# radoslawkrolikowski/financial-market-data-analysis

Measured on AMD Instinct MI355X. Metric: train seq/sec + 3-class acc, biGRU on synthetic order-book, higher is better.
Workload: dtype bf16; 1 GPU; model=biGRU L2 H128 bidirectional, global_batch=8192, seq_len=120, n_features=96, parallelism=dp1, bench_config=repo

## Files before the change

fmda_amd/ops/blas.py:

```python
import os


import torch

_TUNABLE_READY = False


def enable_tunableop() -> bool:
    global _TUNABLE_READY
    if _TUNABLE_READY or not torch.cuda.is_available():
        return _TUNABLE_READY
    try:
        tun = torch.cuda.tunable
        csv = os.path.join(os.path.dirname(__file__), "tunableop_gfx950.csv")
        tune = os.environ.get("FMDA_TUNE", "0") == "1"
        tun.set_filename(csv, insert_device_ordinal=False)
        tun.enable(True)
        tun.tuning_enable(tune)
        _TUNABLE_READY = True
    except Exception:
        _TUNABLE_READY = False
    return _TUNABLE_READY


def chunked_colsum(dg: torch.Tensor, chunks: int = 48) -> torch.Tensor:
    M, N = dg.shape
    c = chunks
    while c > 1 and M % c != 0:
        c //= 2
    if c <= 1:
        return dg.sum(dim=0, dtype=torch.float32)
    return dg.view(c, M // c, N).sum(dim=1, dtype=torch.float32).sum(dim=0)


def chunked_outer(dg: torch.Tensor, x: torch.Tensor,
                  chunks: int = 64, out_fp32: bool = False) -> torch.Tensor:
    M, N = dg.shape
    K = x.shape[1]
    c = chunks
    while c > 1 and M % c != 0:
        c //= 2
    if c <= 1:
        r = torch.matmul(dg.t(), x)
        return r.float() if out_fp32 else r
    parts = torch.bmm(dg.view(c, M // c, N).transpose(1, 2),
                      x.view(c, M // c, K))
    s = parts.float().sum(dim=0)
    return s if out_fp32 else s.to(dg.dtype)
```

fmda_amd/ops/csrc/bindings.cpp:

```cpp
#include <torch/extension.h>
#include <ATen/hip/HIPContext.h>

#include <vector>

extern "C" int fmda_gru_fwd_launch(int is_bf16, int Hp, const void* gi,
                                   const void* w, const float* bhh, void* out,
                                   float* hlast, int B, int Tseq, int n_dir,
                                   const float* h0, void* out_drop,
                                   unsigned int drop_thr, float drop_scale,
                                   unsigned long long drop_seed,
                                   hipStream_t stream);
extern "C" int fmda_gru_fwd_cs_launch(const void* gi, const void* w,
                                      const float* bhh, void* out,
                                      float* hlast, void* hpub,
                                      unsigned int* cnt, int B, int Tseq,
                                      int n_dir, void* out_drop,
                                      unsigned int drop_thr,
                                      float drop_scale,
                                      unsigned long long drop_seed,
                                      hipStream_t stream);
extern "C" int fmda_gru_bwd_cs_launch(const void* gi, const void* w,
                                      const void* wt, const float* bhh,
                                      const void* out, const void* dout,
                                      const float* dhT, void* dgi, void* dgh,
                                      float* dh0, float* dbhh, void* gpub,
                                      unsigned int* cnt, int B, int Tseq,
                                      int n_dir, unsigned int drop_thr,
                                      float drop_scale,
                                      unsigned long long drop_seed,
                                      hipStream_t stream);
extern "C" int fmda_gru_bwd_launch(int is_bf16, int Hp, const void* gi,
                                   const void* w, const void* wt,
                                   const float* bhh,
                                   const void* out, const void* dout,
                                   const float* dhT, void* dgi, void* dgh,
                                   float* dh0, float* dbhh, int B, int Tseq,
                                   int n_dir, unsigned int drop_thr,
                                   float drop_scale,
                                   unsigned long long drop_seed,
                                   const float* h0, void* dgh0,
                                   hipStream_t stream);
extern "C" int fmda_mfma_selftest_launch(const void* A, const void* Bm,
                                         float* C, hipStream_t stream);
extern "C" int fmda_pool_fwd_launch(int is_bf16, const void* out, float* maxv,
                                    float* avgv, int* amax, int B, int Tseq,
                                    int H, int n_dir, hipStream_t stream);
extern "C" int fmda_pool_bwd_launch(int is_bf16, const float* dmax,
                                    const float* davg, const int* amax,
                                    void* dout, int B, int Tseq, int H,
                                    int n_dir, hipStream_t stream);
extern "C" int fmda_dropout_launch(int is_bf16, const void* x, void* y,
                                   long n, unsigned int thr, float scale,
                                   unsigned long long seed,
                                   hipStream_t stream);
extern "C" int fmda_spatial_dropout_launch(int is_bf16, const void* x,
                                           void* y, long B, long Tlen, long F,
                                           unsigned int thr, float scale,
                                           unsigned long long seed,
                                           hipStream_t stream);
extern "C" int fmda_ingest_row_launch(void* ring, const float* row,
                                      const float* xmin, const float* xrng,
                                      int Tseq, int F, hipStream_t stream);
extern "C" int fmda_pool_concat_launch(int is_bf16, const void* out,
                                       const float* hlast, void* feat, int B,
                                       int Tseq, int H, int Hp, int n_dir,
                                       hipStream_t stream);
extern "C" int fmda_head_sigmoid_launch(int is_bf16, const void* x,
                                        const void* W, const void* bias,
                                        float* probs, int B, int K, int C,
                                        hipStream_t stream);
extern "C" int fmda_head_fwd_launch(int is_bf16, const void* x, const void* W,
                                    const void* bias, const float* y,
                                    const float* wgt, const float* pw,
                                    float* logits, float* sig,
                                    float* loss_sum, int B, int K, int C,
                                    hipStream_t stream);
extern "C" int fmda_head_bwd_launch(int is_bf16, const float* sig,
                                    const float* y, const float* wgt,
                                    const float* pw, const float* gscale,
                                    const void* W, float* dlogits, void* dx,
                                    int B, int K, int C, hipStream_t stream);
extern "C" int fmda_gru_bwd_db_rows(int is_bf16, int Hp, int B,
                                    int column_split);
extern "C" int fmda_gru_db_reduce_launch(const float* part, int rows,
                                         int n_dir, int Hp, float* dbhh,
                                         float* dbih, hipStream_t stream);
extern "C" int fmda_opt_norm2_launch(const void* chunks, int n_chunks,
                                     float* out, hipStream_t stream);
namespace fmda_ckpt {
void save_state_dict(const std::string& path,
                     const std::vector<std::string>& keys,
                     const std::vector<torch::Tensor>& tensors);
std::vector<std::pair<std::string, torch::Tensor>> load_state_dict(
        const std::string& path);
}

extern "C" int fmda_opt_adam_launch(const void* chunks, int n_chunks,
                                    const float* norm2, float clip, float lr,
                                    float beta1, float beta2, float eps,
                                    float bc1, float bc2, hipStream_t stream);

namespace {

void check_common(const torch::Tensor& gi, const torch::Tensor& w,
                  const torch::Tensor& bhh, int& B, int& T, int& n_dir,
                  int& Hp, bool& is_bf16) {
    TORCH_CHECK(gi.is_cuda() && w.is_cuda() && bhh.is_cuda(),
                "fmda gru: tensors must be on GPU");
    TORCH_CHECK(gi.is_contiguous() && w.is_contiguous() && bhh.is_contiguous(),
                "fmda gru: tensors must be contiguous");
    TORCH_CHECK(gi.dim() == 3 && w.dim() == 3, "fmda gru: bad ranks");
    TORCH_CHECK(w.scalar_type() == gi.scalar_type(), "fmda gru: dtype mismatch");
    TORCH_CHECK(bhh.scalar_type() == torch::kFloat32, "bhh must be fp32");
    n_dir = w.size(0);
    Hp = w.size(2);
    TORCH_CHECK(w.size(1) == 3 * Hp, "w must be (n_dir, 3H, H)");
    B = gi.size(0);
    T = gi.size(1);
    TORCH_CHECK(gi.size(2) == (int64_t)n_dir * 3 * Hp, "gi last dim mismatch");
    TORCH_CHECK(n_dir == 1 || n_dir == 2, "n_dir must be 1 or 2");
    is_bf16 = gi.scalar_type() == torch::kBFloat16;
    TORCH_CHECK(is_bf16 || gi.scalar_type() == torch::kFloat32,
                "fmda gru: dtype must be bf16 or fp32");
    TORCH_CHECK(!(is_bf16 && Hp < 32),
                "fmda gru: bf16 requires Hp >= 32 (MFMA K=32); pad the "
                "hidden size");
}

struct DropParams {
    unsigned int thr;
    float scale;
};

DropParams drop_params(double p) {
    if (!(p > 0.0)) return {0u, 1.0f};
    return {(unsigned int)((float)p * 256.0f), (float)(1.0 / (1.0 - p))};
}

}

std::vector<torch::Tensor> gru_fwd(torch::Tensor gi, torch::Tensor w,
                                   torch::Tensor bhh,
                                   c10::optional<torch::Tensor> h0_opt,
                                   double drop_p, int64_t drop_seed) {
    int B, T, n_dir, Hp;
    bool is_bf16;
    check_common(gi, w, bhh, B, T, n_dir, Hp, is_bf16);
    const float* h0 = nullptr;
    if (h0_opt.has_value()) {
        auto& h = h0_opt.value();
        TORCH_CHECK(h.is_cuda() && h.is_contiguous() &&
                    h.scalar_type() == torch::kFloat32 &&
                    h.sizes() == torch::IntArrayRef({n_dir, B, Hp}),
                    "h0 must be contiguous fp32 (n_dir, B, Hp)");
        h0 = h.data_ptr<float>();
    }
    auto out = torch::empty({B, T, (int64_t)n_dir * Hp}, gi.options());
    auto hlast = torch::empty({n_dir, B, Hp},
                              gi.options().dtype(torch::kFloat32));
    const DropParams dp = drop_params(drop_p);
    const unsigned int drop_thr = dp.thr;
    const float drop_scale = dp.scale;
    torch::Tensor out_drop;
    void* out_drop_ptr = nullptr;
    if (drop_thr != 0u) {
        TORCH_CHECK(is_bf16 && (Hp == 128 || Hp == 512),
                    "fused fwd dropout requires bf16 Hp=128/512");
        TORCH_CHECK(Hp == 128 || h0 == nullptr,
                    "fused fwd dropout with h0 requires Hp=128");
        out_drop = torch::empty_like(out);
        out_drop_ptr = out_drop.data_ptr();
    }
    auto stream = at::hip::getCurrentHIPStream();
    int rc;
    if (is_bf16 && Hp == 512 && h0 == nullptr) {
        const int BR = 256;
        const int GB = (B + BR - 1) / BR;
        const int G = GB * n_dir;
        auto hpub = torch::empty({2, G, BR, (int64_t)Hp}, gi.options());
        auto cnt = torch::zeros({G}, gi.options().dtype(torch::kUInt32));
        rc = fmda_gru_fwd_cs_launch(gi.data_ptr(), w.data_ptr(),
                                    bhh.data_ptr<float>(), out.data_ptr(),
                                    hlast.data_ptr<float>(), hpub.data_ptr(),
                                    (unsigned int*)cnt.data_ptr(), B, T,
                                    n_dir, out_drop_ptr, drop_thr,
                                    drop_scale,
                                    (unsigned long long)drop_seed,
                                    stream.stream());
    } else {
        rc = fmda_gru_fwd_launch(is_bf16 ? 1 : 0, Hp, gi.data_ptr(),
                                 w.data_ptr(), bhh.data_ptr<float>(),
                                 out.data_ptr(), hlast.data_ptr<float>(), B, T,
                                 n_dir, h0, out_drop_ptr, drop_thr,
                                 drop_scale,
                                 (unsigned long long)drop_seed,
                                 stream.stream());
    }
    TORCH_CHECK(rc == 0, "fmda gru_fwd launch failed rc=", rc, " Hp=", Hp);
    if (out_drop_ptr != nullptr)
        return {out, hlast, out_drop};
    return {out, hlast};
}

std::vector<torch::Tensor> gru_bwd(torch::Tensor gi, torch::Tensor w,
                                   torch::Tensor bhh, torch::Tensor out,
                                   torch::Tensor dout, torch::Tensor dhT,
                                   double drop_p, int64_t drop_seed,
                                   c10::optional<torch::Tensor> h0_opt) {
    int B, T, n_dir, Hp;
    bool is_bf16;
    check_common(gi, w, bhh, B, T, n_dir, Hp, is_bf16);
    const float* h0 = nullptr;
    torch::Tensor dgh0;
    void* dgh0_ptr = nullptr;
    if (h0_opt.has_value()) {
        auto& h = h0_opt.value();
        TORCH_CHECK(h.is_cuda() && h.is_contiguous() &&
                    h.scalar_type() == torch::kFloat32 &&
                    h.sizes() == torch::IntArrayRef({n_dir, B, Hp}),
                    "h0 must be contiguous fp32 (n_dir, B, Hp)");
        h0 = h.data_ptr<float>();
        dgh0 = torch::empty({n_dir, B, (int64_t)3 * Hp}, gi.options());
        dgh0_ptr = dgh0.data_ptr();
    }
    TORCH_CHECK(out.is_contiguous() && dout.is_contiguous() &&
                dhT.is_contiguous(), "fmda gru_bwd: tensors must be contiguous");
    TORCH_CHECK(dhT.scalar_type() == torch::kFloat32, "dhT must be fp32");
    TORCH_CHECK(is_bf16 || Hp <= 256,
                "fp32 backward unsupported for Hp > 256 (LDS budget); "
                "train in bf16 for hidden sizes above 256");
    torch::Tensor dgi, dgh;
    if (getenv("FMDA_ZERO_GRADS")) {
        dgi = torch::zeros_like(gi);
        dgh = torch::zeros_like(gi);
    } else {
        dgi = torch::empty_like(gi);
        dgh = torch::empty_like(gi);
    }
    auto dh0 = torch::empty({n_dir, B, Hp},
                            gi.options().dtype(torch::kFloat32));
    const bool column_split = is_bf16 && Hp == 512 && h0 == nullptr;
    const int64_t db_rows = fmda_gru_bwd_db_rows(is_bf16 ? 1 : 0, Hp, B,
                                                 column_split ? 1 : 0);
    auto dbpart = torch::zeros({db_rows, n_dir, 4 * Hp},
                               gi.options().dtype(torch::kFloat32));
    torch::Tensor wt;
    const void* wt_ptr = nullptr;
    if (is_bf16 && (Hp == 128 || Hp == 512)) {
        wt = w.transpose(1, 2).contiguous();
        wt_ptr = wt.data_ptr();
    }
    auto stream = at::hip::getCurrentHIPStream();
    int rc;
    const DropParams dp = drop_params(drop_p);
    if (column_split) {
        const unsigned int cs_thr = dp.thr;
        const float cs_scale = dp.scale;
        const int BR = 256;
        const int GB = (B + BR - 1) / BR;
        const int G = GB * n_dir;
        auto gpub = torch::empty({2, G, BR, (int64_t)3 * Hp}, gi.options());
        auto cnt = torch::zeros({G}, gi.options().dtype(torch::kUInt32));
        rc = fmda_gru_bwd_cs_launch(
            gi.data_ptr(), w.data_ptr(), wt_ptr, bhh.data_ptr<float>(),
            out.data_ptr(), dout.data_ptr(), dhT.data_ptr<float>(),
            dgi.data_ptr(), dgh.data_ptr(), dh0.data_ptr<float>(),
            dbpart.data_ptr<float>(), gpub.data_ptr(),
            (unsigned int*)cnt.data_ptr(), B, T, n_dir, cs_thr, cs_scale,
            (unsigned long long)drop_seed, stream.stream());
    } else {
        const unsigned int drop_thr = dp.thr;
        const float drop_scale = dp.scale;
        TORCH_CHECK(drop_thr == 0u || (is_bf16 && Hp == 128),
                    "fused dropout-backward on this path requires bf16 "
                    "Hp=128");
        rc = fmda_gru_bwd_launch(is_bf16 ? 1 : 0, Hp, gi.data_ptr(),
                                 w.data_ptr(), wt_ptr, bhh.data_ptr<float>(),
                                 out.data_ptr(), dout.data_ptr(),
                                 dhT.data_ptr<float>(), dgi.data_ptr(),
                                 dgh.data_ptr(), dh0.data_ptr<float>(),
                                 dbpart.data_ptr<float>(), B, T,
                                 n_dir, drop_thr, drop_scale,
                                 (unsigned long long)drop_seed, h0, dgh0_ptr,
                                 stream.stream());
    }
    TORCH_CHECK(rc == 0, "fmda gru_bwd launch failed rc=", rc, " Hp=", Hp);
    auto dbhh = torch::empty({n_dir, 3 * Hp},
                             gi.options().dtype(torch::kFloat32));
    auto dbih = torch::empty_like(dbhh);
    rc = fmda_gru_db_reduce_launch(dbpart.data_ptr<float>(), (int)db_rows,
                                   n_dir, Hp, dbhh.data_ptr<float>(),
                                   dbih.data_ptr<float>(), stream.stream());
    TORCH_CHECK(rc == 0, "fmda gru db reduce launch failed");
    if (dgh0_ptr != nullptr)
        return {dgi, dgh, dh0, dbhh, dbih, dgh0};
    return {dgi, dgh, dh0, dbhh, dbih};
}

torch::Tensor mfma_selftest(torch::Tensor A, torch::Tensor Bm) {
    TORCH_CHECK(A.is_cuda() && A.scalar_type() == torch::kBFloat16);
    TORCH_CHECK(A.sizes() == torch::IntArrayRef({16, 32}) &&
                Bm.sizes() == torch::IntArrayRef({32, 16}));
    auto C = torch::empty({16, 16}, A.options().dtype(torch::kFloat32));
    auto stream = at::hip::getCurrentHIPStream();
    int rc = fmda_mfma_selftest_launch(A.contiguous().data_ptr(),
                                       Bm.contiguous().data_ptr(),
                                       C.data_ptr<float>(), stream.stream());
    TORCH_CHECK(rc == 0, "mfma selftest launch failed");
    return C;
}

std::vector<torch::Tensor> pool_fwd(torch::Tensor out, int64_t n_dir) {
    TORCH_CHECK(out.is_cuda() && out.is_contiguous() && out.dim() == 3);
    const bool bf16 = out.scalar_type() == torch::kBFloat16;
    TORCH_CHECK(bf16 || out.scalar_type() == torch::kFloat32);
    const int B = out.size(0), T = out.size(1);
    const int H = out.size(2) / n_dir;
    TORCH_CHECK(H % 2 == 0, "pool_fwd pairs columns: H must be even "
                "(odd H uses the eager path)");
    auto f32 = out.options().dtype(torch::kFloat32);
    auto maxv = torch::empty({B, H}, f32);
    auto avgv = torch::empty({B, H}, f32);
    auto amax = torch::empty({B, H}, out.options().dtype(torch::kInt32));
    auto stream = at::hip::getCurrentHIPStream();
    int rc = fmda_pool_fwd_launch(bf16 ? 1 : 0, out.data_ptr(),
                                  maxv.data_ptr<float>(), avgv.data_ptr<float>(),
                                  amax.data_ptr<int>(), B, T, H, (int)n_dir,
                                  stream.stream());
    TORCH_CHECK(rc == 0, "pool_fwd launch failed");
    return {maxv, avgv, amax};
}

torch::Tensor pool_bwd(torch::Tensor dmax, torch::Tensor davg,
                       torch::Tensor amax, int64_t T, int64_t n_dir,
                       torch::ScalarType dtype) {
    TORCH_CHECK(dmax.is_cuda() && dmax.is_contiguous() && davg.is_contiguous());
    const int B = dmax.size(0), H = dmax.size(1);
    const bool bf16 = dtype == torch::kBFloat16;
    auto dout = torch::empty({B, T, n_dir * H}, dmax.options().dtype(dtype));
    auto stream = at::hip::getCurrentHIPStream();
    int rc = fmda_pool_bwd_launch(bf16 ? 1 : 0, dmax.data_ptr<float>(),
                                  davg.data_ptr<float>(), amax.data_ptr<int>(),
                                  dout.data_ptr(), B, (int)T, H, (int)n_dir,
                                  stream.stream());
    TORCH_CHECK(rc == 0, "pool_bwd launch failed");
    return dout;
}

torch::Tensor fused_clip_adam(torch::Tensor chunks, int64_t n_chunks,
                              double clip, double lr, double beta1,
                              double beta2, double eps, int64_t step) {
    TORCH_CHECK(chunks.is_cuda() && chunks.scalar_type() == torch::kInt64);
    auto f32 = chunks.options().dtype(torch::kFloat32);
    torch::Tensor norm2;
    auto stream = at::hip::getCurrentHIPStream();
    if (clip > 0) {
        auto part = torch::empty({std::min<int64_t>(n_chunks, 2048)}, f32);
        int rc = fmda_opt_norm2_launch(chunks.data_ptr(), (int)n_chunks,
                                       part.data_ptr<float>(),
                                       stream.stream());
        TORCH_CHECK(rc == 0, "opt norm2 launch failed");
        norm2 = part.sum().reshape({1});
    } else {
        norm2 = torch::zeros({1}, f32);
    }
    const float bc1 = 1.0f - powf((float)beta1, (float)step);
    const float bc2 = 1.0f - powf((float)beta2, (float)step);
    int rc = fmda_opt_adam_launch(chunks.data_ptr(), (int)n_chunks,
                                  norm2.data_ptr<float>(), (float)clip,
                                  (float)lr, (float)beta1, (float)beta2,
                                  (float)eps, bc1, bc2, stream.stream());
    TORCH_CHECK(rc == 0, "opt adam launch failed");
    return norm2;
}

std::vector<torch::Tensor> head_loss_fwd(torch::Tensor x, torch::Tensor W,
                                         torch::Tensor b, torch::Tensor y,
                                         torch::Tensor wgt, torch::Tensor pw) {
    TORCH_CHECK(x.is_cuda() && x.is_contiguous() && W.is_contiguous());
    const bool bf16 = x.scalar_type() == torch::kBFloat16;
    const int B = x.size(0), K = x.size(1), C = W.size(0);
    auto f32 = x.options().dtype(torch::kFloat32);
    auto logits = torch::empty({B, C}, f32);
    auto sig = torch::empty({B, C}, f32);
    auto part = torch::empty({((int64_t)B * C + 255) / 256}, f32);
    auto stream = at::hip::getCurrentHIPStream();
    int rc = fmda_head_fwd_launch(
        bf16 ? 1 : 0, x.data_ptr(), W.data_ptr(), b.data_ptr(),
        y.data_ptr<float>(), wgt.data_ptr<float>(), pw.data_ptr<float>(),
        logits.data_ptr<float>(), sig.data_ptr<float>(),
        part.data_ptr<float>(), B, K, C, stream.stream());
    TORCH_CHECK(rc == 0, "head fwd launch failed");
    return {logits, sig, part.sum().reshape({1})};
}

std::vector<torch::Tensor> head_loss_bwd(torch::Tensor sig, torch::Tensor y,
                                         torch::Tensor wgt, torch::Tensor pw,
                                         torch::Tensor gscale,
                                         torch::Tensor W,
                                         torch::ScalarType xdtype) {
    const int B = sig.size(0), C = sig.size(1), K = W.size(1);
    const bool bf16 = xdtype == torch::kBFloat16;
    auto dlogits = torch::empty_like(sig);
    auto dx = torch::empty({B, K}, sig.options().dtype(xdtype));
    auto stream = at::hip::getCurrentHIPStream();
    int rc = fmda_head_bwd_launch(
        bf16 ? 1 : 0, sig.data_ptr<float>(), y.data_ptr<float>(),
        wgt.data_ptr<float>(), pw.data_ptr<float>(),
        gscale.data_ptr<float>(), W.data_ptr(), dlogits.data_ptr<float>(),
        dx.data_ptr(), B, K, C, stream.stream());
    TORCH_CHECK(rc == 0, "head bwd launch failed");
    return {dlogits, dx};
}

torch::Tensor dropout_fused(torch::Tensor x, double p, int64_t seed) {
    TORCH_CHECK(x.is_cuda() && x.is_contiguous() &&
                x.scalar_type() == torch::kBFloat16);
    auto y = torch::empty_like(x);
    auto stream = at::hip::getCurrentHIPStream();
    const DropParams dp = drop_params(p);
    int rc = fmda_dropout_launch(1, x.data_ptr(), y.data_ptr(), x.numel(),
                                 dp.thr, dp.scale, (unsigned long long)seed,
                                 stream.stream());
    TORCH_CHECK(rc == 0, "dropout launch failed");
    return y;
}

torch::Tensor spatial_dropout_fused(torch::Tensor x, double p,
                                    int64_t seed) {
    TORCH_CHECK(x.is_cuda() && x.is_contiguous() && x.dim() == 3 &&
                x.scalar_type() == torch::kBFloat16);
    auto y = torch::empty_like(x);
    auto stream = at::hip::getCurrentHIPStream();
    const DropParams dp = drop_params(p);
    int rc = fmda_spatial_dropout_launch(
        1, x.data_ptr(), y.data_ptr(), x.size(0), x.size(1), x.size(2),
        dp.thr, dp.scale, (unsigned long long)seed, stream.stream());
    TORCH_CHECK(rc == 0, "spatial dropout launch failed");
    return y;
}

void ingest_row(torch::Tensor ring, torch::Tensor row, torch::Tensor xmin,
                torch::Tensor xrng) {
    TORCH_CHECK(ring.is_cuda() && ring.is_contiguous() && ring.dim() == 2 &&
                ring.scalar_type() == torch::kBFloat16,
                "ring must be (T, F) bf16 on GPU");
    TORCH_CHECK(row.is_cuda() && row.is_contiguous() &&
                row.scalar_type() == torch::kFloat32 &&
                row.numel() == ring.size(1));
    TORCH_CHECK(xmin.is_cuda() && xmin.is_contiguous() &&
                xmin.scalar_type() == torch::kFloat32 &&
                xmin.numel() == ring.size(1), "xmin must be fp32 (F) on GPU");
    TORCH_CHECK(xrng.is_cuda() && xrng.is_contiguous() &&
                xrng.scalar_type() == torch::kFloat32 &&
                xrng.numel() == ring.size(1), "xrng must be fp32 (F) on GPU");
    auto stream = at::hip::getCurrentHIPStream();
    int rc = fmda_ingest_row_launch(
        ring.data_ptr(), row.data_ptr<float>(), xmin.data_ptr<float>(),
        xrng.data_ptr<float>(), ring.size(0), ring.size(1), stream.stream());
    TORCH_CHECK(rc == 0, "ingest_row launch failed rc=", rc);
}

torch::Tensor pool_concat_infer(torch::Tensor out, torch::Tensor hlast,
                                int64_t H) {
    TORCH_CHECK(out.is_cuda() && out.is_contiguous() && out.dim() == 3);
    TORCH_CHECK(hlast.is_contiguous() &&
                hlast.scalar_type() == torch::kFloat32);
    const bool bf16 = out.scalar_type() == torch::kBFloat16;
    const int B = out.size(0), T = out.size(1);
    const int n_dir = hlast.size(0);
    const int Hp = hlast.size(2);
    auto feat = torch::empty({B, 3 * H}, out.options());
    auto stream = at::hip::getCurrentHIPStream();
    int rc = fmda_pool_concat_launch(bf16 ? 1 : 0, out.data_ptr(),
                                     hlast.data_ptr<float>(), feat.data_ptr(),
                                     B, T, (int)H, Hp, n_dir,
                                     stream.stream());
    TORCH_CHECK(rc == 0, "pool_concat launch failed");
    return feat;
}

torch::Tensor head_sigmoid(torch::Tensor x, torch::Tensor W,
                           torch::Tensor b) {
    TORCH_CHECK(x.is_cuda() && x.is_contiguous() && W.is_contiguous() &&
                b.is_contiguous());
    TORCH_CHECK(x.scalar_type() == W.scalar_type() &&
                x.scalar_type() == b.scalar_type());
    const bool bf16 = x.scalar_type() == torch::kBFloat16;
    const int B = x.size(0), K = x.size(1), C = W.size(0);
    auto probs = torch::empty({B, C}, x.options().dtype(torch::kFloat32));
    auto stream = at::hip::getCurrentHIPStream();
    int rc = fmda_head_sigmoid_launch(bf16 ? 1 : 0, x.data_ptr(),
                                      W.data_ptr(), b.data_ptr(),
                                      probs.data_ptr<float>(), B, K, C,
                                      stream.stream());
    TORCH_CHECK(rc == 0, "head_sigmoid launch failed");
    return probs;
}

PYBIND11_MODULE(TORCH_EXTENSION_NAME, m) {
    m.def("gru_fwd", &gru_fwd, "fused biGRU recurrence forward (HIP/CDNA4)",
          py::arg("gi"), py::arg("w"), py::arg("bhh"),
          py::arg("h0") = py::none(), py::arg("drop_p") = 0.0,
          py::arg("drop_seed") = 0);
    m.def("gru_bwd", &gru_bwd, "fused biGRU recurrence backward (HIP/CDNA4)",
          py::arg("gi"), py::arg("w"), py::arg("bhh"), py::arg("out"),
          py::arg("dout"), py::arg("dhT"), py::arg("drop_p") = 0.0,
          py::arg("drop_seed") = 0, py::arg("h0") = py::none());
    m.def("mfma_selftest", &mfma_selftest, "mfma fragment layout self-test");
    m.def("dropout_fused", &dropout_fused,
          "counter-based dropout (mask recomputed in backward)");
    m.def("spatial_dropout_fused", &spatial_dropout_fused,
          "channel (Dropout2d) dropout over (B, T, F) without permutes");
    m.def("ingest_row", &ingest_row,
          "streaming ingest: shift GPU window ring + normalize new row");
    m.def("pool_concat_infer", &pool_concat_infer,
          "fused [dirsum(h_last) | max | avg] concat for inference");
    m.def("head_sigmoid", &head_sigmoid,
          "linear head + sigmoid emitting probabilities");
    m.def("pool_fwd", &pool_fwd, "fused dirsum+max/avg pooling forward");
    m.def("pool_bwd", &pool_bwd, "fused pooling backward (d_out assembly)");
    m.def("head_loss_fwd", &head_loss_fwd, "fused head GEMM + BCE loss");
    m.def("head_loss_bwd", &head_loss_bwd, "fused head/loss backward");
    m.def("fused_clip_adam", &fused_clip_adam,
          "fused multi-tensor grad-clip + Adam step");
    m.def("save_state_dict_native", &fmda_ckpt::save_state_dict,
          "write a torch.load-compatible zip state_dict (native C++)");
    m.def("load_state_dict_native", &fmda_ckpt::load_state_dict,
          "read a torch.save zip state_dict (native C++)");
}
```

fmda_amd/ops/csrc/gru_kernels.hip:

```cpp
#include <hip/hip_runtime.h>
#include <hip/hip_bf16.h>

#define FMDA_DEV __device__ __forceinline__

typedef __bf16 bf16x8_t __attribute__((ext_vector_type(8)));
typedef float f32x4_t __attribute__((ext_vector_type(4)));

namespace fmda {

#define FMDA_LOG2E 1.4426950408889634f

FMDA_DEV float fast_exp2(float x) { return __builtin_amdgcn_exp2f(x); }
FMDA_DEV float fast_rcp(float x) { return __builtin_amdgcn_rcpf(x); }

FMDA_DEV float sigmoidf(float x) {
    return fast_rcp(1.0f + fast_exp2(-x * FMDA_LOG2E));
}

FMDA_DEV float fast_tanh(float x) {
    return 1.0f - 2.0f * fast_rcp(1.0f + fast_exp2(2.0f * FMDA_LOG2E * x));
}

template <typename T> FMDA_DEV float to_f32(T v);
template <> FMDA_DEV float to_f32<float>(float v) { return v; }
// ... 1925 lines not shown
                        (const bf16x8_t*)(asrc + (long)row * 3 * Hp + kbase));
                }
#pragma unroll
                for (int j = 0; j < JT; ++j) {
                    const bf16x8_t bfr = *(const bf16x8_t*)&(
                        (const __bf16*)wt_dir)[
                        (long)(ct * CS + j * 16 + (lane & 15)) * 3 * Hp +
                        kbase];
#pragma unroll
                    for (int m = 0; m < MT; ++m)
                        acc2[j][m] = __builtin_amdgcn_mfma_f32_16x16x32_bf16(
                            a[m], bfr, acc2[j][m], 0, 0, 0);
                }
            }
#pragma unroll
            for (int j = 0; j < JT; ++j)
#pragma unroll
                for (int m = 0; m < MT; ++m)
#pragma unroll
                    for (int e = 0; e < 4; ++e)
                        dhcar[j][m][e] += acc2[j][m][e];
        }

        const bool haveh = (u > 0);
        const __hip_bfloat16* hsrc =
            out_b + (long)(rev ? (Tseq - u) : (u - 1)) * n_dir * Hp;
        f32x4_t acc[NCT][MT];
#pragma unroll
        for (int i = 0; i < NCT; ++i)
#pragma unroll
            for (int m = 0; m < MT; ++m) acc[i][m] = f32x4_t{0.f};
        if (haveh) {
            const int arow = lane & 15;
            const int koff = 8 * (lane >> 4);
#pragma unroll
            for (int kk = 0; kk < KK; ++kk) {
                const int kbase = 32 * kk + koff;
                bf16x8_t a[MT];
#pragma unroll
                for (int m = 0; m < MT; ++m) {
                    int row = 16 * (wave + NW * m) + arow;
                    if (row >= rows_valid) row = 0;
                    a[m] = *(const bf16x8_t*)(hsrc + (long)row * out_row +
                                              kbase);
                }
#pragma unroll
                for (int i = 0; i < NCT; ++i) {
                    const bf16x8_t b = *(const bf16x8_t*)&(
                        (const __bf16*)w_s)[(i * 16 + (lane & 15)) * WPITCH +
                                            kbase];
#pragma unroll
                    for (int m = 0; m < MT; ++m)
                        acc[i][m] = __builtin_amdgcn_mfma_f32_16x16x32_bf16(
                            a[m], b, acc[i][m], 0, 0, 0);
                }
            }
        }

        const __hip_bfloat16* do_t = dout_b + (long)tt * n_dir * Hp + ct * CS;
        float keep_dhn[JT][MT][4];
#pragma unroll
        for (int j = 0; j < JT; ++j) {
            const int jj = j * 16 + (lane & 15);
#pragma unroll
            for (int m = 0; m < MT; ++m) {
#pragma unroll
                for (int e = 0; e < 4; ++e) {
                    const int b = 16 * (wave + NW * m) + 4 * (lane >> 4) + e;
                    const bool live = (b < rows_valid);
                    const float gr = acc[j][m][e] + bhh_s[jj];
                    const float gz = acc[JT + j][m][e] + bhh_s[CS + jj];
                    const float hn =
                        acc[2 * JT + j][m][e] + bhh_s[2 * CS + jj];
                    const float ir = (float)((const __bf16*)gi_s)[b * GP + jj];
                    const float iz =
                        (float)((const __bf16*)gi_s)[b * GP + CS + jj];
                    const float in_ =
                        (float)((const __bf16*)gi_s)[b * GP + 2 * CS + jj];
                    const float r = sigmoidf(ir + gr);
                    const float z = sigmoidf(iz + gz);
                    const float n = fast_tanh(in_ + r * hn);
                    const float hprev =
                        (live && haveh)
                            ? (float)hsrc[(long)b * out_row + ct * CS + jj]
                            : 0.0f;
                    float doval =
                        live ? (float)do_t[(long)b * out_row + jj] : 0.0f;
                    if (drop_thr != 0u) {
                        const long o = ((long)(b0 + b) * Tseq + tt) *
                                           n_dir * Hp +
                                       (long)dir * Hp + ct * CS + jj;
                        const unsigned long long rnd =
                            mix64(drop_seed ^ (unsigned long long)(o >> 3));
                        const unsigned int u =
                            (unsigned int)(rnd >> (8 * ((int)o & 7))) & 0xFF;
                        doval = (u < drop_thr) ? 0.0f : doval * drop_scale;
                    }
                    const float dht = dhcar[j][m][e] + doval;
                    const float dz_pre =
                        live ? dht * (hprev - n) * z * (1.0f - z) : 0.0f;
                    const float dn_pre =
                        live ? dht * (1.0f - z) * (1.0f - n * n) : 0.0f;
                    const float dr_pre =
                        live ? dn_pre * hn * r * (1.0f - r) : 0.0f;
                    const float dhn = live ? dn_pre * r : 0.0f;
                    ((__bf16*)gi_s)[b * GP + jj] =
                        (__bf16)__float2bfloat16(dr_pre);
                    ((__bf16*)gi_s)[b * GP + CS + jj] =
                        (__bf16)__float2bfloat16(dz_pre);
                    ((__bf16*)gi_s)[b * GP + 2 * CS + jj] =
                        (__bf16)__float2bfloat16(dn_pre);
                    keep_dhn[j][m][e] = dhn;
                    dhcar[j][m][e] = live ? dht * z : 0.0f;
                    dbacc[j][0] += dr_pre;
                    dbacc[j][1] += dz_pre;
                    dbacc[j][2] += dhn;
                    dbacc[j][3] += dn_pre;
                }
            }
        }
        asm volatile("s_waitcnt lgkmcnt(0)" ::: "memory");
        __syncthreads();

        {
            __hip_bfloat16* dst = dgi_b + (long)tt * n_dir * 3 * Hp;
            for (int g3 = 0; g3 < 3; ++g3)
                store_tile<__hip_bfloat16, BR, NT>(
                    gi_s + g3 * CS, dst + g3 * Hp + ct * CS, CS, GP, gi_row,
                    rows_valid, tid);
        }
        asm volatile("s_waitcnt lgkmcnt(0)" ::: "memory");
        __syncthreads();
#pragma unroll
        for (int j = 0; j < JT; ++j) {
            const int jj = j * 16 + (lane & 15);
#pragma unroll
            for (int m = 0; m < MT; ++m)
#pragma unroll
                for (int e = 0; e < 4; ++e) {
                    const int b = 16 * (wave + NW * m) + 4 * (lane >> 4) + e;
                    ((__bf16*)gi_s)[b * GP + 2 * CS + jj] =
                        (__bf16)__float2bfloat16(keep_dhn[j][m][e]);
                }
        }
        asm volatile("s_waitcnt lgkmcnt(0)" ::: "memory");
        __syncthreads();
        {
            const int sh = rev ? (tt + 1) : (tt - 1);
            if (sh >= 0 && sh < Tseq) {
                __hip_bfloat16* dst = dgh_b + (long)sh * n_dir * 3 * Hp;
                for (int g3 = 0; g3 < 3; ++g3)
                    store_tile<__hip_bfloat16, BR, NT>(
                        gi_s + g3 * CS, dst + g3 * Hp + ct * CS, CS, GP,
                        gi_row, rows_valid, tid);
            } else {
                __hip_bfloat16* dst =
                    dgh_b + (long)(rev ? 0 : (Tseq - 1)) * n_dir * 3 * Hp;
                for (int g3 = 0; g3 < 3; ++g3)
                    store_zero_tile<__hip_bfloat16, BR, NT>(
                        dst + g3 * Hp + ct * CS, CS, gi_row, rows_valid, tid);
            }
            if (u > 0) {
                __hip_bfloat16* dst =
                    pub_base + (long)(u & 1) * ring_stride;
                constexpr int CPR = CS * 2 / 16;
                for (int g3 = 0; g3 < 3; ++g3)
                    for (int c = tid; c < BR * CPR; c += NT) {
                        const int r = c / CPR;
                        const int jc = c % CPR;
                        u32x4_t v = *(const u32x4_t*)((const char*)(gi_s +
                                        g3 * CS) + (long)r * GP * 2 + jc * 16);
                        store16_sc1((char*)(dst + (long)r * 3 * Hp +
                                            g3 * Hp + ct * CS) + jc * 16, v);
                    }
                asm volatile("s_waitcnt vmcnt(0)" ::: "memory");
                __syncthreads();
                if (tid == 0)
                    __hip_atomic_fetch_add(&cnt[g], 1u, __ATOMIC_RELAXED,
                                           __HIP_MEMORY_SCOPE_AGENT);
            }
        }
        if (u > 0)
            stage_gi(rev ? (Tseq - u) : (u - 1));
        asm volatile("s_waitcnt lgkmcnt(0)" ::: "memory");
        __syncthreads();
    }

    {
        float* d0 = dh0 + ((long)dir * B + b0) * Hp + ct * CS;
#pragma unroll
        for (int j = 0; j < JT; ++j) {
            const int jj = j * 16 + (lane & 15);
#pragma unroll
            for (int m = 0; m < MT; ++m)
#pragma unroll
                for (int e = 0; e < 4; ++e) {
                    const int b = 16 * (wave + NW * m) + 4 * (lane >> 4) + e;
                    if (b < rows_valid) d0[(long)b * Hp + jj] = dhcar[j][m][e];
                }
        }
        float* dbrow =
            dbhh + (((long)gb * NW + wave) * n_dir + dir) * 4 * Hp;
#pragma unroll
        for (int j = 0; j < JT; ++j)
#pragma unroll
            for (int q4 = 0; q4 < 4; ++q4) {
                float v = dbacc[j][q4];
                v += __shfl_xor(v, 16);
                v += __shfl_xor(v, 32);
                if ((lane >> 4) == 0)
                    dbrow[q4 * Hp + ct * CS + j * 16 + (lane & 15)] = v;
            }
    }
}


template <typename T>
__global__ void dropout_kernel(const T* __restrict__ x, T* __restrict__ y,
                               long n, unsigned int thr, float scale,
                               unsigned long long seed) {
    const long o = ((long)blockIdx.x * blockDim.x + threadIdx.x) * 8;
    if (o >= n) return;
    const unsigned long long r = mix64(seed ^ (unsigned long long)(o >> 3));
    if (o + 8 <= n) {
        T v[8];
        *(chunk16*)v = *(const chunk16*)(x + o);
#pragma unroll
        for (int k = 0; k < 8; ++k) {
            const unsigned int u = (unsigned int)(r >> (8 * k)) & 0xFF;
            v[k] = (u < thr) ? from_f32<T>(0.0f)
                             : from_f32<T>(to_f32<T>(v[k]) * scale);
        }
        *(chunk16*)(y + o) = *(const chunk16*)v;
    } else {
        for (long i = o; i < n; ++i) {
            const unsigned int u =
                (unsigned int)(r >> (8 * (i - o))) & 0xFF;
            y[i] = (u < thr) ? from_f32<T>(0.0f)
                             : from_f32<T>(to_f32<T>(x[i]) * scale);
        }
    }
}

extern "C" int fmda_dropout_launch(int is_bf16, const void* x, void* y,
                                   long n, unsigned int thr, float scale,
                                   unsigned long long seed,
                                   hipStream_t stream) {
    const long threads = (n + 7) / 8;
    const dim3 grid((threads + 255) / 256);
    if (is_bf16)
        dropout_kernel<__hip_bfloat16><<<grid, 256, 0, stream>>>(
            (const __hip_bfloat16*)x, (__hip_bfloat16*)y, n, thr, scale,
            seed);
    else
        return -2;
    return hipGetLastError() == hipSuccess ? 0 : -1;
}

template <typename T>
__global__ void spatial_dropout_kernel(const T* __restrict__ x,
                                       T* __restrict__ y, long n, long TF,
                                       int F, unsigned int thr, float scale,
                                       unsigned long long seed) {
    const long o = ((long)blockIdx.x * blockDim.x + threadIdx.x) * 8;
    if (o >= n) return;
    const int cnt = (int)((o + 8 <= n) ? 8 : (n - o));
    T v[8];
    if (cnt == 8)
        *(chunk16*)v = *(const chunk16*)(x + o);
    else
        for (int k = 0; k < cnt; ++k) v[k] = x[o + k];
#pragma unroll
    for (int k = 0; k < 8; ++k) {
        if (k >= cnt) break;
        const long i = o + k;
        const long c = (i / TF) * F + (i % F);
        const unsigned long long r =
            mix64(seed ^ (unsigned long long)(c >> 3));
        const unsigned int u = (unsigned int)(r >> (8 * ((int)c & 7))) & 0xFF;
        v[k] = (u < thr) ? from_f32<T>(0.0f)
                         : from_f32<T>(to_f32<T>(v[k]) * scale);
    }
    if (cnt == 8)
        *(chunk16*)(y + o) = *(const chunk16*)v;
    else
        for (int k = 0; k < cnt; ++k) y[o + k] = v[k];
}

extern "C" int fmda_spatial_dropout_launch(int is_bf16, const void* x,
                                           void* y, long B, long Tlen, long F,
                                           unsigned int thr, float scale,
                                           unsigned long long seed,
                                           hipStream_t stream) {
    if (!is_bf16) return -2;
    const long n = B * Tlen * F;
    const long threads = (n + 7) / 8;
    const dim3 grid((threads + 255) / 256);
    spatial_dropout_kernel<__hip_bfloat16><<<grid, 256, 0, stream>>>(
        (const __hip_bfloat16*)x, (__hip_bfloat16*)y, n, Tlen * F, (int)F,
        thr, scale, seed);
    return hipGetLastError() == hipSuccess ? 0 : -1;
}

template <typename T>
__global__ void pool_fwd_kernel(const T* __restrict__ out,
                                float* __restrict__ maxv,
                                float* __restrict__ avgv,
                                int* __restrict__ amax, int B, int Tseq,
                                int H, int n_dir) {
    const int idx = blockIdx.x * blockDim.x + threadIdx.x;
    const int HP2 = H / 2;
    if (idx >= B * HP2) return;
    const int b = idx / HP2;
    const int h2 = (idx % HP2) * 2;
    const int HD = n_dir * H;
    const T* p = out + (long)b * Tseq * HD + h2;
    float mx0 = -3.4e38f, mx1 = -3.4e38f, s0 = 0.0f, s1 = 0.0f;
    int im0 = 0, im1 = 0;
    for (int t = 0; t < Tseq; ++t) {
        const T* pt = p + (long)t * HD;
        struct alignas(2 * sizeof(T)) Pair { T x, y; };
        const Pair v2 = *(const Pair*)pt;
        float v0 = to_f32<T>(v2.x), v1 = to_f32<T>(v2.y);
        if (n_dir == 2) {
            const Pair w2 = *(const Pair*)(pt + H);
            v0 += to_f32<T>(w2.x);
            v1 += to_f32<T>(w2.y);
        }
        s0 += v0; s1 += v1;
        if (v0 > mx0) { mx0 = v0; im0 = t; }
        if (v1 > mx1) { mx1 = v1; im1 = t; }
    }
    const int o = b * H + h2;
    maxv[o] = mx0; maxv[o + 1] = mx1;
    avgv[o] = s0 / (float)Tseq; avgv[o + 1] = s1 / (float)Tseq;
    amax[o] = im0; amax[o + 1] = im1;
}

template <typename T>
__global__ void pool_bwd_kernel(const float* __restrict__ dmax,
                                const float* __restrict__ davg,
                                const int* __restrict__ amax,
                                T* __restrict__ dout, int B, int Tseq, int H,
                                int n_dir) {
    const int idx = blockIdx.x * blockDim.x + threadIdx.x;
    if (idx >= B * H) return;
    const int b = idx / H;
    const int h = idx % H;
    const int HD = n_dir * H;
    const float ga = davg[idx] / (float)Tseq;
    const float gm = dmax[idx];
    const int im = amax[idx];
    T* p = dout + (long)b * Tseq * HD + h;
    for (int t = 0; t < Tseq; ++t) {
        const float g = ga + (t == im ? gm : 0.0f);
        p[(long)t * HD] = from_f32<T>(g);
        if (n_dir == 2) p[(long)t * HD + H] = from_f32<T>(g);
    }
}

__global__ void pool_fwd_oct_kernel(const __hip_bfloat16* __restrict__ out,
                                    float* __restrict__ maxv,
                                    float* __restrict__ avgv,
                                    int* __restrict__ amax, int B, int Tseq,
                                    int H, int n_dir) {
    const int idx = blockIdx.x * blockDim.x + threadIdx.x;
    const int H8 = H / 8;
    if (idx >= B * H8) return;
    const int b = idx / H8;
    const int h8 = (idx % H8) * 8;
    const int HD = n_dir * H;
    const __hip_bfloat16* p = out + (long)b * Tseq * HD + h8;
    float mx[8], s[8];
    int im[8];
#pragma unroll
    for (int k = 0; k < 8; ++k) { mx[k] = -3.4e38f; s[k] = 0.0f; im[k] = 0; }
    for (int t = 0; t < Tseq; ++t) {
        const __hip_bfloat16* pt = p + (long)t * HD;
        bf16x8_t v = *(const bf16x8_t*)pt;
        bf16x8_t w;
        if (n_dir == 2) w = *(const bf16x8_t*)(pt + H);
#pragma unroll
        for (int k = 0; k < 8; ++k) {
            float x = (float)((const __bf16*)&v)[k];
            if (n_dir == 2) x += (float)((const __bf16*)&w)[k];
            s[k] += x;
            if (x > mx[k]) { mx[k] = x; im[k] = t; }
        }
    }
    const int o = b * H + h8;
#pragma unroll
    for (int k = 0; k < 8; ++k) {
        maxv[o + k] = mx[k];
        avgv[o + k] = s[k] / (float)Tseq;
        amax[o + k] = im[k];
    }
}

__global__ void pool_bwd_oct_kernel(const float* __restrict__ dmax,
                                    const float* __restrict__ davg,
                                    const int* __restrict__ amax,
                                    __hip_bfloat16* __restrict__ dout,
                                    int B, int Tseq, int H, int n_dir) {
    const int idx = blockIdx.x * blockDim.x + threadIdx.x;
    const int H8 = H / 8;
    if (idx >= B * H8) return;
    const int b = idx / H8;
    const int h8 = (idx % H8) * 8;
    const int o = b * H + h8;
    float ga[8], gm[8];
    int im[8];
#pragma unroll
    for (int k = 0; k < 8; ++k) {
        ga[k] = davg[o + k] / (float)Tseq;
        gm[k] = dmax[o + k];
        im[k] = amax[o + k];
    }
    const int HD = n_dir * H;
    __hip_bfloat16* p = dout + (long)b * Tseq * HD + h8;
    for (int t = 0; t < Tseq; ++t) {
        bf16x8_t v;
#pragma unroll
        for (int k = 0; k < 8; ++k)
            ((__bf16*)&v)[k] =
                (__bf16)__float2bfloat16(ga[k] + (t == im[k] ? gm[k] : 0.0f));
        *(bf16x8_t*)(p + (long)t * HD) = v;
        if (n_dir == 2) *(bf16x8_t*)(p + (long)t * HD + H) = v;
    }
}

template <typename T>
__global__ void pool_fwd_small_kernel(const T* __restrict__ out,
                                      float* __restrict__ maxv,
                                      float* __restrict__ avgv,
                                      int* __restrict__ amax, int B, int Tseq,
                                      int H, int n_dir) {
    const int HP2 = H / 2;
    const int wave = threadIdx.x >> 6;
    const int lane = threadIdx.x & 63;
    const int idx = blockIdx.x * (blockDim.x >> 6) + wave;
    if (idx >= B * HP2) return;
    const int b = idx / HP2;
    const int h2 = (idx % HP2) * 2;
    const int HD = n_dir * H;
    const T* p = out + (long)b * Tseq * HD + h2;
    float mx0 = -3.4e38f, mx1 = -3.4e38f, s0 = 0.0f, s1 = 0.0f;
    int im0 = Tseq, im1 = Tseq;
    for (int t = lane; t < Tseq; t += 64) {
        const T* pt = p + (long)t * HD;
        struct alignas(2 * sizeof(T)) Pair { T x, y; };
        const Pair v2 = *(const Pair*)pt;
        float v0 = to_f32<T>(v2.x), v1 = to_f32<T>(v2.y);
        if (n_dir == 2) {
            const Pair w2 = *(const Pair*)(pt + H);
            v0 += to_f32<T>(w2.x);
            v1 += to_f32<T>(w2.y);
        }
        s0 += v0; s1 += v1;
        if (v0 > mx0) { mx0 = v0; im0 = t; }
        if (v1 > mx1) { mx1 = v1; im1 = t; }
    }
#pragma unroll
    for (int d = 1; d < 64; d <<= 1) {
        const float omx0 = __shfl_xor(mx0, d), omx1 = __shfl_xor(mx1, d);
        const int oim0 = __shfl_xor(im0, d), oim1 = __shfl_xor(im1, d);
        s0 += __shfl_xor(s0, d);
        s1 += __shfl_xor(s1, d);
        if (omx0 > mx0 || (omx0 == mx0 && oim0 < im0)) { mx0 = omx0; im0 = oim0; }
        if (omx1 > mx1 || (omx1 == mx1 && oim1 < im1)) { mx1 = omx1; im1 = oim1; }
    }
    if (lane == 0) {
        const int o = b * H + h2;
        maxv[o] = mx0; maxv[o + 1] = mx1;
        avgv[o] = s0 / (float)Tseq; avgv[o + 1] = s1 / (float)Tseq;
        amax[o] = im0; amax[o + 1] = im1;
    }
}

extern "C" int fmda_pool_fwd_launch(int is_bf16, const void* out, float* maxv,
                                    float* avgv, int* amax, int B, int Tseq,
                                    int H, int n_dir, hipStream_t stream) {
    const int n = B * (H / 2);
    if (n < 4096) {
        const dim3 grid((n + 3) / 4);
        if (is_bf16)
            pool_fwd_small_kernel<__hip_bfloat16><<<grid, 256, 0, stream>>>(
                (const __hip_bfloat16*)out, maxv, avgv, amax, B, Tseq, H,
                n_dir);
        else
            pool_fwd_small_kernel<float><<<grid, 256, 0, stream>>>(
                (const float*)out, maxv, avgv, amax, B, Tseq, H, n_dir);
        return hipGetLastError() == hipSuccess ? 0 : -1;
    }
    if (is_bf16 && H % 8 == 0) {
        const int n8 = B * (H / 8);
        pool_fwd_oct_kernel<<<dim3((n8 + 255) / 256), 256, 0, stream>>>(
            (const __hip_bfloat16*)out, maxv, avgv, amax, B, Tseq, H, n_dir);
        return hipGetLastError() == hipSuccess ? 0 : -1;
    }
    const dim3 grid((n + 255) / 256);
    if (is_bf16)
        pool_fwd_kernel<__hip_bfloat16><<<grid, 256, 0, stream>>>(
            (const __hip_bfloat16*)out, maxv, avgv, amax, B, Tseq, H, n_dir);
    else
        pool_fwd_kernel<float><<<grid, 256, 0, stream>>>(
            (const float*)out, maxv, avgv, amax, B, Tseq, H, n_dir);
    return hipGetLastError() == hipSuccess ? 0 : -1;
}

extern "C" int fmda_pool_bwd_launch(int is_bf16, const float* dmax,
                                    const float* davg, const int* amax,
                                    void* dout, int B, int Tseq, int H,
                                    int n_dir, hipStream_t stream) {
    const int n = B * H;
    if (is_bf16 && H % 8 == 0 && B * (H / 8) >= 4096) {
        const int n8 = B * (H / 8);
        pool_bwd_oct_kernel<<<dim3((n8 + 255) / 256), 256, 0, stream>>>(
            dmax, davg, amax, (__hip_bfloat16*)dout, B, Tseq, H, n_dir);
        return hipGetLastError() == hipSuccess ? 0 : -1;
    }
    const dim3 grid((n + 255) / 256);
    if (is_bf16)
        pool_bwd_kernel<__hip_bfloat16><<<grid, 256, 0, stream>>>(
            dmax, davg, amax, (__hip_bfloat16*)dout, B, Tseq, H, n_dir);
    else
        pool_bwd_kernel<float><<<grid, 256, 0, stream>>>(
            dmax, davg, amax, (float*)dout, B, Tseq, H, n_dir);
    return hipGetLastError() == hipSuccess ? 0 : -1;
}


__global__ void ingest_row_kernel(__hip_bfloat16* __restrict__ ring,
                                  const float* __restrict__ row,
                                  const float* __restrict__ xmin,
                                  const float* __restrict__ xrng,
                                  int Tseq, int F) {
    const int n = (Tseq - 1) * F;
    const int tid = threadIdx.x;
    __hip_bfloat16 keep[48];
    int cnt = 0;
    for (int i = tid; i < n; i += blockDim.x) keep[cnt++] = ring[i + F];
    __syncthreads();
    cnt = 0;
    for (int i = tid; i < n; i += blockDim.x) ring[i] = keep[cnt++];
    for (int f = tid; f < F; f += blockDim.x)
        ring[n + f] = __float2bfloat16((row[f] - xmin[f]) / xrng[f]);
}

extern "C" int fmda_ingest_row_launch(void* ring, const float* row,
                                      const float* xmin, const float* xrng,
                                      int Tseq, int F, hipStream_t stream) {
    const int n = (Tseq - 1) * F;
    if (n > 48 * 1024) return -5;
    ingest_row_kernel<<<1, 1024, 0, stream>>>(
        (__hip_bfloat16*)ring, row, xmin, xrng, Tseq, F);
    return hipGetLastError() == hipSuccess ? 0 : -1;
}

template <typename T>
__global__ void pool_concat_infer_kernel(const T* __restrict__ out,
                                         const float* __restrict__ hlast,
                                         T* __restrict__ feat, int B,
                                         int Tseq, int H, int Hp, int n_dir) {
    const int HP2 = H / 2;
    const int wave = threadIdx.x >> 6;
    const int lane = threadIdx.x & 63;
    const int idx = blockIdx.x * (blockDim.x >> 6) + wave;
    if (idx >= B * HP2) return;
    const int b = idx / HP2;
    const int h2 = (idx % HP2) * 2;
    const int HD = n_dir * H;
    const T* p = out + (long)b * Tseq * HD + h2;
    float mx0 = -3.4e38f, mx1 = -3.4e38f, s0 = 0.0f, s1 = 0.0f;
    for (int t = lane; t < Tseq; t += 64) {
        const T* pt = p + (long)t * HD;
        struct alignas(2 * sizeof(T)) Pair { T x, y; };
        const Pair v2 = *(const Pair*)pt;
        float v0 = to_f32<T>(v2.x), v1 = to_f32<T>(v2.y);
        if (n_dir == 2) {
            const Pair w2 = *(const Pair*)(pt + H);
            v0 += to_f32<T>(w2.x);
            v1 += to_f32<T>(w2.y);
        }
        s0 += v0; s1 += v1;
        if (v0 > mx0) mx0 = v0;
        if (v1 > mx1) mx1 = v1;
    }
#pragma unroll
    for (int d = 1; d < 64; d <<= 1) {
        const float omx0 = __shfl_xor(mx0, d), omx1 = __shfl_xor(mx1, d);
        s0 += __shfl_xor(s0, d);
        s1 += __shfl_xor(s1, d);
        if (omx0 > mx0) mx0 = omx0;
        if (omx1 > mx1) mx1 = omx1;
    }
    if (lane == 0) {
        float hl0 = hlast[(long)b * Hp + h2];
        float hl1 = hlast[(long)b * Hp + h2 + 1];
        if (n_dir == 2) {
            hl0 += hlast[((long)B + b) * Hp + h2];
            hl1 += hlast[((long)B + b) * Hp + h2 + 1];
        }
        T* fr = feat + (long)b * 3 * H;
        fr[h2] = from_f32<T>(hl0);
        fr[h2 + 1] = from_f32<T>(hl1);
        fr[H + h2] = from_f32<T>(mx0);
        fr[H + h2 + 1] = from_f32<T>(mx1);
        fr[2 * H + h2] = from_f32<T>(s0 / (float)Tseq);
        fr[2 * H + h2 + 1] = from_f32<T>(s1 / (float)Tseq);
    }
}

extern "C" int fmda_pool_concat_launch(int is_bf16, const void* out,
                                       const float* hlast, void* feat, int B,
                                       int Tseq, int H, int Hp, int n_dir,
                                       hipStream_t stream) {
    const int n = B * (H / 2);
    const dim3 grid((n + 3) / 4);
    if (is_bf16)
        pool_concat_infer_kernel<__hip_bfloat16><<<grid, 256, 0, stream>>>(
            (const __hip_bfloat16*)out, hlast, (__hip_bfloat16*)feat, B,
            Tseq, H, Hp, n_dir);
    else
        pool_concat_infer_kernel<float><<<grid, 256, 0, stream>>>(
            (const float*)out, hlast, (float*)feat, B, Tseq, H, Hp, n_dir);
    return hipGetLastError() == hipSuccess ? 0 : -1;
}

template <typename T>
__global__ void head_sigmoid_kernel(const T* __restrict__ x,
                                    const T* __restrict__ W,
                                    const T* __restrict__ bias,
                                    float* __restrict__ probs, int B, int K,
                                    int C) {
    const int wave = threadIdx.x >> 6;
    const int lane = threadIdx.x & 63;
    const int idx = blockIdx.x * (blockDim.x >> 6) + wave;
    if (idx >= B * C) return;
    const int b = idx / C, c = idx % C;
    const T* xr = x + (long)b * K;
    const T* wr = W + (long)c * K;
    float acc = 0.0f;
    for (int k = lane; k < K; k += 64)
        acc += to_f32<T>(xr[k]) * to_f32<T>(wr[k]);
#pragma unroll
    for (int d = 1; d < 64; d <<= 1) acc += __shfl_xor(acc, d);
    if (lane == 0) probs[idx] = sigmoidf(acc + to_f32<T>(bias[c]));
}

extern "C" int fmda_head_sigmoid_launch(int is_bf16, const void* x,
                                        const void* W, const void* bias,
                                        float* probs, int B, int K, int C,
                                        hipStream_t stream) {
    const int n = B * C;
    const dim3 grid((n + 3) / 4);
    if (is_bf16)
        head_sigmoid_kernel<__hip_bfloat16><<<grid, 256, 0, stream>>>(
            (const __hip_bfloat16*)x, (const __hip_bfloat16*)W,
            (const __hip_bfloat16*)bias, probs, B, K, C);
    else
        head_sigmoid_kernel<float><<<grid, 256, 0, stream>>>(
            (const float*)x, (const float*)W, (const float*)bias, probs, B,
            K, C);
    return hipGetLastError() == hipSuccess ? 0 : -1;
}

template <typename T>
__global__ void head_loss_fwd_kernel(const T* __restrict__ x,
                                     const T* __restrict__ W,
                                     const T* __restrict__ bias,
                                     const float* __restrict__ y,
                                     const float* __restrict__ wgt,
                                     const float* __restrict__ pw,
                                     float* __restrict__ logits,
                                     float* __restrict__ sig,
                                     float* __restrict__ loss_sum, int B,
                                     int K, int C) {
    const int idx = blockIdx.x * blockDim.x + threadIdx.x;
    float l = 0.0f;
    if (idx < B * C) {
        const int r = idx / C, c = idx % C;
        const T* xr = x + (long)r * K;
        const T* wr = W + (long)c * K;
        float acc = to_f32<T>(bias[c]);
        for (int k = 0; k < K; ++k)
            acc += to_f32<T>(xr[k]) * to_f32<T>(wr[k]);
        logits[idx] = acc;
        const float s = sigmoidf(acc);
        sig[idx] = s;
        const float yy = y[idx];
        const float m = acc > 0.0f ? acc : 0.0f;
        const float lse = m + __builtin_logf(fast_exp2(-m * FMDA_LOG2E) +
                                             fast_exp2((acc - m) * FMDA_LOG2E));
        const float log_s = acc - lse;
        const float log_1ms = -lse;
        l = -wgt[c] * (pw[c] * yy * log_s + (1.0f - yy) * log_1ms);
    }
    __shared__ float red[4];
    float v = l;
    v += __shfl_xor(v, 1); v += __shfl_xor(v, 2); v += __shfl_xor(v, 4);
    v += __shfl_xor(v, 8); v += __shfl_xor(v, 16); v += __shfl_xor(v, 32);
    if ((threadIdx.x & 63) == 0) red[threadIdx.x >> 6] = v;
    __syncthreads();
    if (threadIdx.x == 0) {
        float t = 0.0f;
        for (int w = 0; w < (int)(blockDim.x >> 6); ++w) t += red[w];
        loss_sum[blockIdx.x] = t;
    }
}

template <typename T>
__global__ void head_loss_bwd_kernel(const float* __restrict__ sig,
                                     const float* __restrict__ y,
                                     const float* __restrict__ wgt,
                                     const float* __restrict__ pw,
                                     const float* __restrict__ gscale,
                                     const T* __restrict__ W,
                                     float* __restrict__ dlogits,
                                     T* __restrict__ dx, int B, int K, int C) {
    const int idx = blockIdx.x * blockDim.x + threadIdx.x;
    if (idx >= B * K) return;
    const int r = idx / K, k = idx % K;
    const float g = *gscale / (float)(B * C);
    float acc = 0.0f;
    for (int c = 0; c < C; ++c) {
        const float s = sig[r * C + c];
        const float yy = y[r * C + c];
        const float dl = g * wgt[c] * (s * (1.0f - yy + pw[c] * yy) -
                                       pw[c] * yy);
        if (k == 0) dlogits[r * C + c] = dl;
        acc += dl * to_f32<T>(W[(long)c * K + k]);
    }
    dx[idx] = from_f32<T>(acc);
}

extern "C" int fmda_head_fwd_launch(int is_bf16, const void* x, const void* W,
                                    const void* bias, const float* y,
                                    const float* wgt, const float* pw,
                                    float* logits, float* sig,
                                    float* loss_sum, int B, int K, int C,
                                    hipStream_t stream) {
    const int n = B * C;
    const dim3 grid((n + 255) / 256);
    if (is_bf16)
        head_loss_fwd_kernel<__hip_bfloat16><<<grid, 256, 0, stream>>>(
            (const __hip_bfloat16*)x, (const __hip_bfloat16*)W,
            (const __hip_bfloat16*)bias, y, wgt, pw, logits, sig, loss_sum,
            B, K, C);
    else
        head_loss_fwd_kernel<float><<<grid, 256, 0, stream>>>(
            (const float*)x, (const float*)W, (const float*)bias, y, wgt, pw,
            logits, sig, loss_sum, B, K, C);
    return hipGetLastError() == hipSuccess ? 0 : -1;
}

extern "C" int fmda_head_bwd_launch(int is_bf16, const float* sig,
                                    const float* y, const float* wgt,
                                    const float* pw, const float* gscale,
                                    const void* W, float* dlogits, void* dx,
                                    int B, int K, int C, hipStream_t stream) {
    const int n = B * K;
    const dim3 grid((n + 255) / 256);
    if (is_bf16)
        head_loss_bwd_kernel<__hip_bfloat16><<<grid, 256, 0, stream>>>(
            sig, y, wgt, pw, gscale, (const __hip_bfloat16*)W, dlogits,
            (__hip_bfloat16*)dx, B, K, C);
    else
        head_loss_bwd_kernel<float><<<grid, 256, 0, stream>>>(
            sig, y, wgt, pw, gscale, (const float*)W, dlogits, (float*)dx,
            B, K, C);
    return hipGetLastError() == hipSuccess ? 0 : -1;
}

__global__ void mfma_selftest_kernel(const __hip_bfloat16* __restrict__ A,
                                     const __hip_bfloat16* __restrict__ Bm,
                                     float* __restrict__ C) {
    const int lane = threadIdx.x & 63;
    bf16x8_t a, b;
    const __bf16* ap = (const __bf16*)A;
    const __bf16* bp = (const __bf16*)Bm;
#pragma unroll
    for (int e = 0; e < 8; ++e) {
        a[e] = ap[(lane & 15) * 32 + 8 * (lane >> 4) + e];
        b[e] = bp[(8 * (lane >> 4) + e) * 16 + (lane & 15)];
    }
    f32x4_t acc = f32x4_t{0.f};
    acc = __builtin_amdgcn_mfma_f32_16x16x32_bf16(a, b, acc, 0, 0, 0);
#pragma unroll
    for (int v = 0; v < 4; ++v)
        C[(4 * (lane >> 4) + v) * 16 + (lane & 15)] = acc[v];
}


struct LaunchCfg { int bt; bool wlds; int nt; bool hoist; };

static inline LaunchCfg fwd_cfg(bool bf16, int Hp) {
    if (bf16) {
        if (Hp <= 64) return {32, true, 256, false};
        if (Hp == 128) return {32, false, 512, true};
        if (Hp == 256) return {32, false, 512, false};
        return {16, false, 512, false};
    }
    if (Hp <= 128) return {32, false, 256, false};
    return {16, false, 256, false};
}
static inline LaunchCfg bwd_cfg(bool bf16, int Hp) {
    if (bf16) {
        if (Hp <= 64) return {32, true, 256, false};
        if (Hp == 128) return {32, false, 512, true};
        if (Hp == 256) return {32, false, 512, false};
        return {16, false, 512, false};
    }
    if (Hp <= 128) return {32, false, 256, false};
    return {16, false, 256, false};
}

static inline size_t fwd_lds_bytes(bool bf16, int Hp, int bt, bool wlds) {
    const size_t es = bf16 ? 2 : 4;
    const size_t pade = 16 / es;
    const size_t wp = Hp + pade, gp3 = 3 * Hp + pade, hfp = Hp + 4;
    size_t s = 0;
    if (wlds) s += es * 3 * Hp * wp;
    s += 4 * (size_t)bt * hfp;
    if (bf16) s += 2 * (size_t)bt * wp;
    s += es * (size_t)bt * gp3;
    s += 4 * (size_t)3 * Hp;
    return s;
}
static inline size_t bwd_lds_bytes(bool bf16, int Hp, int bt, bool wlds) {
    const size_t es = bf16 ? 2 : 4;
// ... 376 lines not shown
```

fmda_amd/ops/interface.py:

```python
import os
from typing import List, Optional, Tuple

import torch

from . import load_extension
from .blas import chunked_colsum, chunked_outer, enable_tunableop

_ALLOWED_HP = [32, 64, 128, 256, 512]


def _pad_h(H: int) -> int:
    for hp in _ALLOWED_HP:
        if H <= hp:
            return hp
    raise ValueError(f"hidden size {H} > {_ALLOWED_HP[-1]} not supported")


def _pad_gate_rows(w: torch.Tensor, H: int, Hp: int) -> torch.Tensor:
    if H == Hp:
        return w
    shape = list(w.shape)
    shape[0] = 3 * Hp
    out = w.new_zeros(shape)
    for g in range(3):
        out[g * Hp:g * Hp + H] = w[g * H:(g + 1) * H]
    return out


def _pad_cols(w: torch.Tensor, H: int, Hp: int) -> torch.Tensor:
    if H == Hp:
        return w
    shape = list(w.shape)
    shape[-1] = Hp
    out = w.new_zeros(shape)
    out[..., :H] = w
    return out


class _GRURecurrence(torch.autograd.Function):

    @staticmethod
    def forward(ctx, gi, w, bhh, h0=None):
        ext = load_extension()
        gi = gi.contiguous()
        w = w.contiguous()
        bhh32 = bhh.to(torch.float32).contiguous()
        h0c = (h0.detach().to(torch.float32).contiguous()
               if h0 is not None else None)
        out, h_last = ext.gru_fwd(gi, w, bhh32, h0c)
        ctx.save_for_backward(gi, w, bhh32, out)
        ctx.h0 = h0c
        return out, h_last

    @staticmethod
    def backward(ctx, d_out, d_hlast):
        ext = load_extension()
        gi, w, bhh32, out = ctx.saved_tensors
        h0c = ctx.h0
        B, T, _ = gi.shape
        n_dir, threeHp, Hp = w.shape
        d_out = d_out.contiguous().to(gi.dtype)
        d_hlast = d_hlast.contiguous().to(torch.float32)
        res = ext.gru_bwd(gi, w, bhh32, out, d_out, d_hlast, 0.0, 0, h0c)
        dgi, dgh, dh0_out, dbhh, _dbih = res[:5]
        dgh0 = res[5] if len(res) > 5 else None

        cross = chunked_outer(dgh.reshape(-1, n_dir * threeHp),
                              out.reshape(-1, n_dir * Hp))
        dw = torch.empty_like(w)
        for d in range(n_dir):
            dw[d] = cross[d * threeHp:(d + 1) * threeHp,
                          d * Hp:(d + 1) * Hp]
            if dgh0 is not None:
                dw[d] += (dgh0[d].float().t() @ h0c[d]).to(dw.dtype)
        dh0_grad = dh0_out if h0c is not None else None
        return dgi, dw, dbhh, dh0_grad


def gru_directions(gi: torch.Tensor, w: torch.Tensor, bhh: torch.Tensor,
                   h0: Optional[torch.Tensor] = None
                   ) -> Tuple[torch.Tensor, torch.Tensor]:
    return _GRURecurrence.apply(gi, w, bhh, h0)


class _IHProjection(torch.autograd.Function):

    @staticmethod
    def forward(ctx, x2d, w, b):
        ctx.save_for_backward(x2d, w)
        return torch.addmm(b, x2d, w.t())

    @staticmethod
    def backward(ctx, dgi):
        x2d, w = ctx.saved_tensors
        dgi = dgi.contiguous()
        dx = dw = db = None
        if ctx.needs_input_grad[0]:
            dx = torch.matmul(dgi, w)
        if ctx.needs_input_grad[1]:
            dw = chunked_outer(dgi, x2d)
        if ctx.needs_input_grad[2]:
            db = chunked_colsum(dgi).to(dgi.dtype)
        return dx, dw, db


class _FusedDropout(torch.autograd.Function):

    @staticmethod
    def forward(ctx, x, p, seed):
        ext = load_extension()
        ctx.p = p
        ctx.seed = seed
        return ext.dropout_fused(x.contiguous(), p, seed)

    @staticmethod
    def backward(ctx, dy):
        ext = load_extension()
        return ext.dropout_fused(dy.contiguous(), ctx.p, ctx.seed), None, None


def fused_dropout(x: torch.Tensor, p: float) -> torch.Tensor:
    if not (x.is_cuda and x.dtype == torch.bfloat16 and 0.0 < p < 1.0):
        return torch.nn.functional.dropout(x, p=p, training=True)
    seed = int(torch.empty((), dtype=torch.int64).random_())
    return _FusedDropout.apply(x, p, seed)


class _FusedSpatialDropout(torch.autograd.Function):

    @staticmethod
    def forward(ctx, x, p, seed):
        ext = load_extension()
        ctx.p = p
        ctx.seed = seed
        return ext.spatial_dropout_fused(x.contiguous(), p, seed)

    @staticmethod
    def backward(ctx, dy):
        ext = load_extension()
        return (ext.spatial_dropout_fused(dy.contiguous(), ctx.p, ctx.seed),
                None, None)


def fused_spatial_dropout(x: torch.Tensor, p: float) -> torch.Tensor:
    if not (x.is_cuda and x.dtype == torch.bfloat16 and 0.0 < p < 1.0):
        y = torch.nn.functional.dropout2d(
            x.permute(0, 2, 1).unsqueeze(-1), p=p, training=True)
        return y.squeeze(-1).permute(0, 2, 1)
    seed = int(torch.empty((), dtype=torch.int64).random_())
    return _FusedSpatialDropout.apply(x, p, seed)


class _DirSumPool(torch.autograd.Function):

    @staticmethod
    def forward(ctx, out, n_dir):
        ext = load_extension()
        out = out.contiguous()
        maxv, avgv, amax = ext.pool_fwd(out, n_dir)
        ctx.save_for_backward(amax)
        ctx.meta = (out.shape[1], n_dir, out.dtype)
        return maxv.to(out.dtype), avgv.to(out.dtype)

    @staticmethod
    def backward(ctx, dmax, davg):
        ext = load_extension()
        (amax,) = ctx.saved_tensors
        T, n_dir, dtype = ctx.meta
        dout = ext.pool_bwd(dmax.float().contiguous(),
                            davg.float().contiguous(), amax, T, n_dir, dtype)
        return dout, None


def dirsum_pool(out: torch.Tensor, n_dir: int):
    return _DirSumPool.apply(out, n_dir)


class _HeadLoss(torch.autograd.Function):

    @staticmethod
    def forward(ctx, x2d, W, b, y, wgt, pw):
        ext = load_extension()
        x2d = x2d.contiguous()
        logits, sig, loss_sum = ext.head_loss_fwd(
            x2d, W.contiguous(), b.contiguous(), y.contiguous(),
            wgt.contiguous(), pw.contiguous())
        B, C = logits.shape
        loss = (loss_sum / float(B * C)).reshape(())
        ctx.save_for_backward(x2d, W, y, wgt, pw, sig)
        ctx.mark_non_differentiable(logits)
        return loss, logits

    @staticmethod
    def backward(ctx, dloss, _dlogits):
        ext = load_extension()
        x2d, W, y, wgt, pw, sig = ctx.saved_tensors
        dlogits, dx = ext.head_loss_bwd(sig, y, wgt, pw,
                                        dloss.reshape(1).float().contiguous(),
                                        W, x2d.dtype)
        dl = dlogits.to(x2d.dtype)
        dW = chunked_outer(dl, x2d)
        db = dlogits.sum(dim=0).to(W.dtype)
        return dx, dW, db, None, None, None


def fused_head_loss(x2d, weight, bias, y, wgt, pw):
    Wc = weight.to(x2d.dtype)
    bc = bias.to(x2d.dtype)
    return _HeadLoss.apply(x2d, Wc, bc, y.float(), wgt.float(), pw.float())


def _unpad_gate_rows(w, H, Hp):
    if H == Hp:
        return w
    return torch.cat([w[g * Hp:g * Hp + H] for g in range(3)], dim=0)


class _BiGRULayer(torch.autograd.Function):

    @staticmethod
    def forward(ctx, x, Hp, w_ih0, w_hh0, b_ih0, b_hh0,
                w_ih1, w_hh1, b_ih1, b_hh1, out_drop_p=0.0,
                out_drop_seed=0, h0=None):
        ext = load_extension()
        D = 2 if w_ih1 is not None else 1
        H = w_hh0.shape[1]
        dtype = x.dtype
        B, T, F = x.shape
        with torch.no_grad():
            w_ihs = [_pad_gate_rows(w_ih0, H, Hp)]
            w_hhs = [_pad_cols(_pad_gate_rows(w_hh0, H, Hp), H, Hp)]
            b_ihs = [_pad_gate_rows(b_ih0, H, Hp)]
            b_hhs = [_pad_gate_rows(b_hh0, H, Hp)]
            if D == 2:
                w_ihs.append(_pad_gate_rows(w_ih1, H, Hp))
                w_hhs.append(_pad_cols(_pad_gate_rows(w_hh1, H, Hp), H, Hp))
                b_ihs.append(_pad_gate_rows(b_ih1, H, Hp))
                b_hhs.append(_pad_gate_rows(b_hh1, H, Hp))
            w_ih_cat = torch.cat(w_ihs, dim=0).to(dtype)
            b_ih_cat = torch.cat(b_ihs, dim=0).to(dtype)
            w_hh_cat = torch.stack(w_hhs, dim=0).to(dtype)
            b_hh_cat = torch.stack(b_hhs, dim=0).float()
        x2d = x.reshape(B * T, F)
        gi = torch.addmm(b_ih_cat, x2d, w_ih_cat.t()).view(B, T, -1)
        h0c = h0.detach().contiguous() if h0 is not None else None
        res = ext.gru_fwd(gi, w_hh_cat, b_hh_cat, h0c, out_drop_p,
                          out_drop_seed)
        out, h_last = res[0], res[1]
        ctx.save_for_backward(x2d, w_ih_cat, w_hh_cat, b_hh_cat, gi, out)
        ctx.h0 = h0c
        ctx.meta = (D, H, Hp, out_drop_p, out_drop_seed)
        ctx.set_materialize_grads(False)
        if len(res) > 2:
            return out, h_last, res[2]
        return out, h_last

    @staticmethod
    def backward(ctx, d_out, d_hlast, d_outdrop=None):
        ext = load_extension()
        x2d, w_ih_cat, w_hh_cat, b_hh_cat, gi, out = ctx.saved_tensors
        D, H, Hp, drop_p, drop_seed = ctx.meta
        need_dx = ctx.needs_input_grad[0]
        if drop_p > 0:
            assert d_out is None, "unexpected grad on raw out with fused dropout"
            d_out = d_outdrop
        if d_out is None:
            d_out = torch.zeros_like(out)
        if d_hlast is None:
            d_hlast = out.new_zeros(
                (w_hh_cat.shape[0], out.shape[0], Hp), dtype=torch.float32)
        d_out = d_out.contiguous().to(gi.dtype)
        d_hlast = d_hlast.contiguous().float()
        h0c = ctx.h0
        res = ext.gru_bwd(gi, w_hh_cat, b_hh_cat, out, d_out, d_hlast,
                          drop_p, drop_seed, h0c)
        dgi, dgh, dh0_out, dbhh, dbih = res[:5]
        dgh0 = res[5] if len(res) > 5 else None
        M = dgi.shape[0] * dgi.shape[1]

        cross = chunked_outer(dgh.reshape(M, -1), out.reshape(M, -1),
                              out_fp32=True)
        if dgh0 is not None:
            for d in range(D):
                cross[d * 3 * Hp:(d + 1) * 3 * Hp,
                      d * Hp:(d + 1) * Hp] += dgh0[d].float().t() @ h0c[d]
        dwih_cat = chunked_outer(dgi.reshape(M, -1), x2d, out_fp32=True)
        dx = None
        if need_dx:
            dx = torch.matmul(dgi.reshape(M, -1), w_ih_cat)
            dx = dx.view(dgi.shape[0], dgi.shape[1], -1)

        grads = []
        for d in range(D):
            dwih = dwih_cat[d * 3 * Hp:(d + 1) * 3 * Hp]
            dwhh = cross[d * 3 * Hp:(d + 1) * 3 * Hp,
                         d * Hp:(d + 1) * Hp].contiguous()
            grads.append((
                _unpad_gate_rows(dwih, H, Hp),
                _unpad_gate_rows(dwhh, H, Hp)[:, :H],
                _unpad_gate_rows(dbih[d], H, Hp),
                _unpad_gate_rows(dbhh[d], H, Hp)))
        if D == 1:
            grads.append((None, None, None, None))
        (a0, b0, c0, e0), (a1, b1, c1, e1) = grads
        dh0_grad = dh0_out if h0c is not None else None
        return (dx, None, a0, b0, c0, e0, a1, b1, c1, e1, None, None,
                dh0_grad)



_PACK_EPOCH = 0


def _packed_inference_weights(gru_module, layer, params, Hp, H, dtype):
    key = f"_fmda_pack_l{layer}_{dtype}_{params[0][0].device}"
    flat = [t for four in params for t in four]
    versions = (_PACK_EPOCH,) + tuple(t._version for t in flat)
    ent = getattr(gru_module, key, None)
    if ent is not None and ent[0] == versions:
        return ent[1]
    w_ihs, w_hhs, b_ihs, b_hhs = [], [], [], []
    for (w_ih, w_hh, b_ih, b_hh) in params:
        w_ihs.append(_pad_gate_rows(w_ih, H, Hp))
        w_hhs.append(_pad_cols(_pad_gate_rows(w_hh, H, Hp), H, Hp))
        b_ihs.append(_pad_gate_rows(b_ih, H, Hp))
        b_hhs.append(_pad_gate_rows(b_hh, H, Hp))
    packed = (torch.cat(w_ihs, dim=0).to(dtype),
              torch.cat(b_ihs, dim=0).to(dtype),
              torch.stack(w_hhs, dim=0).to(dtype).contiguous(),
              torch.stack(b_hhs, dim=0).float().contiguous())
    setattr(gru_module, key, (versions, packed))
    return packed


def bigru_stack(x: torch.Tensor, gru_module: torch.nn.GRU, n_layers: int,
                bidirectional: bool, dropout_p: float, training: bool,
                hidden: Optional[torch.Tensor] = None
                ) -> Tuple[torch.Tensor, torch.Tensor]:
    enable_tunableop()
    D = 2 if bidirectional else 1
    H = gru_module.hidden_size
    Hp = _pad_h(H)

    h0_layers = [None] * n_layers
    if hidden is not None:
        B = x.shape[0]
        assert hidden.shape == (n_layers * D, B, H), \
            f"hidden must be ({n_layers * D}, {B}, {H})"
        hid32 = hidden.float()
        for layer in range(n_layers):
            h0_layers[layer] = _pad_cols(
                hid32[layer * D:(layer + 1) * D], H, Hp).contiguous()

    h_n_parts: List[torch.Tensor] = []
    inp = x
    for layer in range(n_layers):
        p = {}
        for d, sfx_d in enumerate(["", "_reverse"][:D]):
            sfx = f"l{layer}{sfx_d}"
            p[d] = (getattr(gru_module, f"weight_ih_{sfx}"),
                    getattr(gru_module, f"weight_hh_{sfx}"),
                    getattr(gru_module, f"bias_ih_{sfx}"),
                    getattr(gru_module, f"bias_hh_{sfx}"))
        drop_here = (training and dropout_p > 0 and layer < n_layers - 1)
        defer = (drop_here and Hp == H and Hp in (128, 512)
                 and x.dtype == torch.bfloat16 and x.is_cuda
                 and (Hp == 128 or (h0_layers[layer] is None
                      and os.environ.get("FMDA_CS_DROP", "1") != "0")))
        seed = (int(torch.empty((), dtype=torch.int64).random_())
                if defer else 0)
        dp = (dropout_p, seed) if defer else (0.0, 0)

        h0_l = h0_layers[layer]
        dropped_pad = None
        if not training and not torch.is_grad_enabled():
            ext = load_extension()
            w_ih_cat, b_ih_cat, w_hh_cat, b_hh_cat = _packed_inference_weights(
                gru_module, layer, [p[d] for d in range(D)], Hp, H, x.dtype)
            B, T, F = inp.shape
            gi = torch.addmm(b_ih_cat, inp.reshape(B * T, F),
                             w_ih_cat.t()).view(B, T, -1)
            out_pad, h_last = ext.gru_fwd(gi, w_hh_cat, b_hh_cat, h0_l)
        elif D == 2:
            res = _BiGRULayer.apply(inp, Hp, *p[0], *p[1], *dp, h0_l)
            out_pad, h_last = res[0], res[1]
            dropped_pad = res[2] if len(res) > 2 else None
        else:
            res = _BiGRULayer.apply(inp, Hp, *p[0],
                                    None, None, None, None, *dp, h0_l)
            out_pad, h_last = res[0], res[1]
            dropped_pad = res[2] if len(res) > 2 else None

        if Hp == H:
            out = out_pad
        elif D == 2:
            out = torch.cat([out_pad[..., :H], out_pad[..., Hp:Hp + H]],
                            dim=-1)
        else:
            out = out_pad[..., :H]
        h_n_parts.append(h_last[:, :, :H].to(x.dtype))

        inp = out
        if drop_here:
            if defer:
                inp = dropped_pad
            else:
                inp = fused_dropout(inp, dropout_p)

    h_n = torch.cat(h_n_parts, dim=0)
    return inp, h_n
```

setup.py:

```python
import os

from setuptools import setup

os.environ.setdefault("PYTORCH_ROCM_ARCH", "gfx950")

from torch.utils.cpp_extension import BuildExtension, CUDAExtension

setup(
    name="fmda_amd",
    version="0.1.0",
    packages=["fmda_amd", "fmda_amd.data", "fmda_amd.models", "fmda_amd.ops",
              "fmda_amd.parallel", "fmda_amd.runtime"],
    ext_modules=[
        CUDAExtension(
            name="fmda_amd.ops._fmda_hip",
            sources=[
                "fmda_amd/ops/csrc/bindings.cpp",
                "fmda_amd/ops/csrc/gru_kernels.hip",
                "fmda_amd/ops/csrc/optim_kernels.hip",
                "fmda_amd/ops/csrc/checkpoint.cpp",
            ],
            extra_compile_args={
                "cxx": ["-O3", "-std=c++17"],
                "nvcc": ["-O3", "-std=c++17"],
            },
        )
    ],
    cmdclass={"build_ext": BuildExtension.with_options(no_python_abi_suffix=False)},
)
```

Before: 1.055 million seq/s.

## Fuse GRU weight packing, grad finalization, head and pooling glue into native kernels

```diff
diff --git a/fmda_amd/ops/blas.py b/fmda_amd/ops/blas.py
--- a/fmda_amd/ops/blas.py
+++ b/fmda_amd/ops/blas.py
@@ -35,15 +35,21 @@
 
 def chunked_outer(dg: torch.Tensor, x: torch.Tensor,
                   chunks: int = 64, out_fp32: bool = False) -> torch.Tensor:
+    parts = chunked_outer_parts(dg, x, chunks)
+    if parts.shape[0] == 1:
+        return parts[0].float() if out_fp32 else parts[0]
+    s = parts.float().sum(dim=0)
+    return s if out_fp32 else s.to(dg.dtype)
+
+
+def chunked_outer_parts(dg: torch.Tensor, x: torch.Tensor,
+                        chunks: int = 64) -> torch.Tensor:
     M, N = dg.shape
     K = x.shape[1]
     c = chunks
     while c > 1 and M % c != 0:
         c //= 2
     if c <= 1:
-        r = torch.matmul(dg.t(), x)
-        return r.float() if out_fp32 else r
-    parts = torch.bmm(dg.view(c, M // c, N).transpose(1, 2),
-                      x.view(c, M // c, K))
-    s = parts.float().sum(dim=0)
-    return s if out_fp32 else s.to(dg.dtype)
+        return torch.matmul(dg.t(), x).unsqueeze(0)
+    return torch.bmm(dg.view(c, M // c, N).transpose(1, 2),
+                     x.view(c, M // c, K))
diff --git a/fmda_amd/ops/csrc/bindings.cpp b/fmda_amd/ops/csrc/bindings.cpp
--- a/fmda_amd/ops/csrc/bindings.cpp
+++ b/fmda_amd/ops/csrc/bindings.cpp
@@ -42,13 +42,15 @@
                                    hipStream_t stream);
 extern "C" int fmda_mfma_selftest_launch(const void* A, const void* Bm,
                                          float* C, hipStream_t stream);
-extern "C" int fmda_pool_fwd_launch(int is_bf16, const void* out, float* maxv,
-                                    float* avgv, int* amax, int B, int Tseq,
-                                    int H, int n_dir, hipStream_t stream);
-extern "C" int fmda_pool_bwd_launch(int is_bf16, const float* dmax,
-                                    const float* davg, const int* amax,
+extern "C" int fmda_pool_fwd_launch(int is_bf16, const void* out, void* maxv,
+                                    void* avgv, int* amax, int B, int Tseq,
+                                    int H, int n_dir, int act_io,
+                                    hipStream_t stream);
+extern "C" int fmda_pool_bwd_launch(int is_bf16, const void* dmax,
+                                    const void* davg, const int* amax,
                                     void* dout, int B, int Tseq, int H,
-                                    int n_dir, hipStream_t stream);
+                                    int n_dir, int act_io, long ld_max,
+                                    long ld_avg, hipStream_t stream);
 extern "C" int fmda_dropout_launch(int is_bf16, const void* x, void* y,
                                    long n, unsigned int thr, float scale,
                                    unsigned long long seed,
@@ -87,6 +89,28 @@
                                          float* dbih, hipStream_t stream);
 extern "C" int fmda_opt_norm2_launch(const void* chunks, int n_chunks,
                                      float* out, hipStream_t stream);
+extern "C" int fmda_pack_gru_layer_launch(
+        int is_bf16, const float* const* masters, void* w_ih_cat,
+        void* b_ih_cat, void* w_hh_cat, float* b_hh_cat, void* wt, int D,
+        int H, int Hp, int F, hipStream_t stream);
+extern "C" int fmda_finalize_gru_wgrads_launch(
+        int part_bf16, const void* part_ih, int c_ih, const void* part_hh,
+        int c_hh, float* const* grads, int D, int H, int Hp, int F,
+        hipStream_t stream);
+extern "C" int fmda_head_fwd_master_launch(
+        int is_bf16, const void* x, const float* W, const float* bias,
+        const float* y, const float* wgt, const float* pw, float* logits,
+        float* sig, float* loss_sum, int B, int K, int C,
+        hipStream_t stream);
+extern "C" int fmda_head_bwd_master_launch(
+        int is_bf16, const float* sig, const float* y, const float* wgt,
+        const float* pw, const float* gscale, const float* W,
+        float* dlogits, void* dx, int B, int K, int C, hipStream_t stream);
+extern "C" int fmda_head_wgrads_slabs(int B);
+extern "C" int fmda_head_wgrads_launch(
+        int is_bf16, const float* dlogits, const void* x, float* dw_part,
+        float* db_part, float* dW, float* db, int B, int K, int C,
+        hipStream_t stream);
 namespace fmda_ckpt {
 void save_state_dict(const std::string& path,
                      const std::vector<std::string>& keys,
@@ -206,7 +230,8 @@
                                    torch::Tensor bhh, torch::Tensor out,
                                    torch::Tensor dout, torch::Tensor dhT,
                                    double drop_p, int64_t drop_seed,
-                                   c10::optional<torch::Tensor> h0_opt) {
+                                   c10::optional<torch::Tensor> h0_opt,
+                                   c10::optional<torch::Tensor> wt_opt) {
     int B, T, n_dir, Hp;
     bool is_bf16;
     check_common(gi, w, bhh, B, T, n_dir, Hp, is_bf16);
@@ -247,7 +272,16 @@
     torch::Tensor wt;
     const void* wt_ptr = nullptr;
     if (is_bf16 && (Hp == 128 || Hp == 512)) {
-        wt = w.transpose(1, 2).contiguous();
+        if (wt_opt.has_value()) {
+            wt = wt_opt.value();
+            TORCH_CHECK(wt.is_cuda() && wt.is_contiguous() &&
+                        wt.scalar_type() == w.scalar_type() &&
+                        wt.sizes() == torch::IntArrayRef(
+                            {n_dir, Hp, (int64_t)3 * Hp}),
+                        "wt must be contiguous (n_dir, Hp, 3Hp) in w's dtype");
+        } else {
+            wt = w.transpose(1, 2).contiguous();
+        }
         wt_ptr = wt.data_ptr();
     }
     auto stream = at::hip::getCurrentHIPStream();
@@ -310,7 +344,8 @@
     return C;
 }
 
-std::vector<torch::Tensor> pool_fwd(torch::Tensor out, int64_t n_dir) {
+std::vector<torch::Tensor> pool_fwd(torch::Tensor out, int64_t n_dir,
+                                    bool act_dtype) {
     TORCH_CHECK(out.is_cuda() && out.is_contiguous() && out.dim() == 3);
     const bool bf16 = out.scalar_type() == torch::kBFloat16;
     TORCH_CHECK(bf16 || out.scalar_type() == torch::kFloat32);
@@ -318,15 +353,17 @@
     const int H = out.size(2) / n_dir;
     TORCH_CHECK(H % 2 == 0, "pool_fwd pairs columns: H must be even "
                 "(odd H uses the eager path)");
-    auto f32 = out.options().dtype(torch::kFloat32);
-    auto maxv = torch::empty({B, H}, f32);
-    auto avgv = torch::empty({B, H}, f32);
+    const bool act_io = act_dtype && bf16;
+    auto pooled = out.options().dtype(act_io ? torch::kBFloat16
+                                             : torch::kFloat32);
+    auto maxv = torch::empty({B, H}, pooled);
+    auto avgv = torch::empty({B, H}, pooled);
     auto amax = torch::empty({B, H}, out.options().dtype(torch::kInt32));
     auto stream = at::hip::getCurrentHIPStream();
     int rc = fmda_pool_fwd_launch(bf16 ? 1 : 0, out.data_ptr(),
-                                  maxv.data_ptr<float>(), avgv.data_ptr<float>(),
+                                  maxv.data_ptr(), avgv.data_ptr(),
                                   amax.data_ptr<int>(), B, T, H, (int)n_dir,
-                                  stream.stream());
+                                  act_io ? 1 : 0, stream.stream());
     TORCH_CHECK(rc == 0, "pool_fwd launch failed");
     return {maxv, avgv, amax};
 }
@@ -334,14 +371,27 @@
 torch::Tensor pool_bwd(torch::Tensor dmax, torch::Tensor davg,
                        torch::Tensor amax, int64_t T, int64_t n_dir,
                        torch::ScalarType dtype) {
-    TORCH_CHECK(dmax.is_cuda() && dmax.is_contiguous() && davg.is_contiguous());
+    TORCH_CHECK(dmax.is_cuda() && davg.is_cuda() && dmax.dim() == 2 &&
+                davg.sizes() == dmax.sizes() && amax.sizes() == dmax.sizes() &&
+                amax.is_contiguous(), "pool_bwd: shape mismatch");
     const int B = dmax.size(0), H = dmax.size(1);
+    TORCH_CHECK((H == 1 || (dmax.stride(1) == 1 && davg.stride(1) == 1)) &&
+                (B == 1 || (dmax.stride(0) >= H && davg.stride(0) >= H)),
+                "pool_bwd: dmax / davg need unit column stride");
     const bool bf16 = dtype == torch::kBFloat16;
+    const bool act_io = bf16 && dmax.scalar_type() == torch::kBFloat16;
+    TORCH_CHECK(dmax.scalar_type() == davg.scalar_type() &&
+                (act_io || dmax.scalar_type() == torch::kFloat32),
+                "pool_bwd: dmax / davg must both be fp32, or both bf16 with "
+                "bf16 activations");
     auto dout = torch::empty({B, T, n_dir * H}, dmax.options().dtype(dtype));
     auto stream = at::hip::getCurrentHIPStream();
-    int rc = fmda_pool_bwd_launch(bf16 ? 1 : 0, dmax.data_ptr<float>(),
-                                  davg.data_ptr<float>(), amax.data_ptr<int>(),
+    int rc = fmda_pool_bwd_launch(bf16 ? 1 : 0, dmax.data_ptr(),
+                                  davg.data_ptr(), amax.data_ptr<int>(),
                                   dout.data_ptr(), B, (int)T, H, (int)n_dir,
+                                  act_io ? 1 : 0,
+                                  B == 1 ? H : (long)dmax.stride(0),
+                                  B == 1 ? H : (long)davg.stride(0),
                                   stream.stream());
     TORCH_CHECK(rc == 0, "pool_bwd launch failed");
     return dout;
@@ -498,6 +548,170 @@
     return probs;
 }
 
+namespace {
+
+void check_f32_cuda(const torch::Tensor& t, const char* what) {
+    TORCH_CHECK(t.is_cuda() && t.is_contiguous() &&
+                t.scalar_type() == torch::kFloat32,
+                what, " must be a contiguous fp32 GPU tensor");
+}
+
+bool compute_dtype_is_bf16(torch::ScalarType dtype) {
+    TORCH_CHECK(dtype == torch::kBFloat16 || dtype == torch::kFloat32,
+                "compute dtype must be bf16 or fp32");
+    return dtype == torch::kBFloat16;
+}
+
+}
+
+std::vector<torch::Tensor> pack_gru_layer(std::vector<torch::Tensor> masters,
+                                          int64_t Hp,
+                                          torch::ScalarType dtype) {
+    TORCH_CHECK(masters.size() == 4 || masters.size() == 8,
+                "pack_gru_layer: 4 masters per direction, 1 or 2 directions");
+    const int64_t D = masters.size() / 4;
+    for (auto& t : masters) check_f32_cuda(t, "pack_gru_layer: master");
+    TORCH_CHECK(masters[0].dim() == 2 && masters[1].dim() == 2,
+                "pack_gru_layer: bad weight ranks");
+    const int64_t H = masters[1].size(1), F = masters[0].size(1);
+    TORCH_CHECK(H <= Hp, "pack_gru_layer: H > Hp");
+    const float* ptrs[8] = {};
+    for (int64_t d = 0; d < D; ++d) {
+        TORCH_CHECK(masters[4 * d].sizes() == torch::IntArrayRef({3 * H, F}) &&
+                    masters[4 * d + 1].sizes() ==
+                        torch::IntArrayRef({3 * H, H}) &&
+                    masters[4 * d + 2].sizes() == torch::IntArrayRef({3 * H}) &&
+                    masters[4 * d + 3].sizes() == torch::IntArrayRef({3 * H}),
+                    "pack_gru_layer: master shapes disagree");
+        for (int k = 0; k < 4; ++k)
+            ptrs[4 * d + k] = masters[4 * d + k].data_ptr<float>();
+    }
+    const bool bf16 = compute_dtype_is_bf16(dtype);
+    auto opt = masters[0].options().dtype(dtype);
+    auto w_ih_cat = torch::empty({D * 3 * Hp, F}, opt);
+    auto b_ih_cat = torch::empty({D * 3 * Hp}, opt);
+    auto w_hh_cat = torch::empty({D, 3 * Hp, Hp}, opt);
+    auto b_hh_cat = torch::empty({D, 3 * Hp}, masters[0].options());
+    auto wt = torch::empty({D, Hp, 3 * Hp}, opt);
+    auto stream = at::hip::getCurrentHIPStream();
+    int rc = fmda_pack_gru_layer_launch(
+        bf16 ? 1 : 0, ptrs, w_ih_cat.data_ptr(), b_ih_cat.data_ptr(),
+        w_hh_cat.data_ptr(), b_hh_cat.data_ptr<float>(), wt.data_ptr(),
+        (int)D, (int)H, (int)Hp, (int)F, stream.stream());
+    TORCH_CHECK(rc == 0, "pack_gru_layer launch failed");
+    return {w_ih_cat, b_ih_cat, w_hh_cat, b_hh_cat, wt};
+}
+
+std::vector<torch::Tensor> finalize_gru_wgrads(torch::Tensor part_ih,
+                                               torch::Tensor part_hh,
+                                               int64_t D, int64_t H,
+                                               int64_t Hp) {
+    TORCH_CHECK(part_ih.is_cuda() && part_hh.is_cuda() &&
+                part_ih.is_contiguous() && part_hh.is_contiguous() &&
+                part_ih.dim() == 3 && part_hh.dim() == 3,
+                "finalize_gru_wgrads: partials must be contiguous (c, N, K) "
+                "GPU tensors");
+    TORCH_CHECK(part_ih.scalar_type() == part_hh.scalar_type(),
+                "finalize_gru_wgrads: partial dtypes disagree");
+    const bool bf16 = compute_dtype_is_bf16(part_ih.scalar_type());
+    TORCH_CHECK((D == 1 || D == 2) && H >= 1 && H <= Hp,
+                "finalize_gru_wgrads: bad D / H / Hp");
+    const int64_t F = part_ih.size(2);
+    TORCH_CHECK(part_ih.size(1) == D * 3 * Hp &&
+                part_hh.size(1) == D * 3 * Hp && part_hh.size(2) == D * Hp,
+                "finalize_gru_wgrads: partial shapes disagree with D / Hp");
+    auto f32 = part_ih.options().dtype(torch::kFloat32);
+    std::vector<torch::Tensor> grads;
+    float* ptrs[4] = {};
+    for (int64_t d = 0; d < D; ++d) {
+        grads.push_back(torch::empty({3 * H, F}, f32));
+        grads.push_back(torch::empty({3 * H, H}, f32));
+        ptrs[2 * d] = grads[2 * d].data_ptr<float>();
+        ptrs[2 * d + 1] = grads[2 * d + 1].data_ptr<float>();
+    }
+    auto stream = at::hip::getCurrentHIPStream();
+    int rc = fmda_finalize_gru_wgrads_launch(
+        bf16 ? 1 : 0, part_ih.data_ptr(), (int)part_ih.size(0),
+        part_hh.data_ptr(), (int)part_hh.size(0), ptrs, (int)D, (int)H,
+        (int)Hp, (int)F, stream.stream());
+    TORCH_CHECK(rc == 0, "finalize_gru_wgrads launch failed");
+    return grads;
+}
+
+std::vector<torch::Tensor> head_loss_fwd_master(
+        torch::Tensor x, torch::Tensor W, torch::Tensor b, torch::Tensor y,
+        torch::Tensor wgt, torch::Tensor pw) {
+    TORCH_CHECK(x.is_cuda() && x.is_contiguous() && x.dim() == 2);
+    const bool bf16 = compute_dtype_is_bf16(x.scalar_type());
+    check_f32_cuda(W, "head W"); check_f32_cuda(b, "head b");
+    check_f32_cuda(y, "head y"); check_f32_cuda(wgt, "head weight");
+    check_f32_cuda(pw, "head pos_weight");
+    const int B = x.size(0), K = x.size(1), C = W.size(0);
+    TORCH_CHECK(W.size(1) == K && b.numel() == C && y.numel() == (int64_t)B * C
+                && wgt.numel() == C && pw.numel() == C,
+                "head_loss_fwd_master: shape mismatch");
+    auto f32 = x.options().dtype(torch::kFloat32);
+    auto logits = torch::empty({B, C}, f32);
+    auto sig = torch::empty({B, C}, f32);
+    auto part = torch::empty({((int64_t)B * C + 255) / 256}, f32);
+    auto stream = at::hip::getCurrentHIPStream();
+    int rc = fmda_head_fwd_master_launch(
+        bf16 ? 1 : 0, x.data_ptr(), W.data_ptr<float>(), b.data_ptr<float>(),
+        y.data_ptr<float>(), wgt.data_ptr<float>(), pw.data_ptr<float>(),
+        logits.data_ptr<float>(), sig.data_ptr<float>(),
+        part.data_ptr<float>(), B, K, C, stream.stream());
+    TORCH_CHECK(rc == 0, "head fwd (master) launch failed");
+    return {logits, sig, part.sum().reshape({1})};
+}
+
+std::vector<torch::Tensor> head_loss_bwd_master(
+        torch::Tensor sig, torch::Tensor y, torch::Tensor wgt,
+        torch::Tensor pw, torch::Tensor gscale, torch::Tensor W,
+        torch::ScalarType xdtype) {
+    check_f32_cuda(sig, "head sig"); check_f32_cuda(y, "head y");
+    check_f32_cuda(wgt, "head weight"); check_f32_cuda(pw, "head pos_weight");
+    check_f32_cuda(gscale, "head gscale"); check_f32_cuda(W, "head W");
+    const int B = sig.size(0), C = sig.size(1), K = W.size(1);
+    TORCH_CHECK(W.size(0) == C && y.numel() == sig.numel() &&
+                wgt.numel() == C && pw.numel() == C && gscale.numel() == 1,
+                "head_loss_bwd_master: shape mismatch");
+    const bool bf16 = compute_dtype_is_bf16(xdtype);
+    auto dlogits = torch::empty_like(sig);
+    auto dx = torch::empty({B, K}, sig.options().dtype(xdtype));
+    auto stream = at::hip::getCurrentHIPStream();
+    int rc = fmda_head_bwd_master_launch(
+        bf16 ? 1 : 0, sig.data_ptr<float>(), y.data_ptr<float>(),
+        wgt.data_ptr<float>(), pw.data_ptr<float>(),
+        gscale.data_ptr<float>(), W.data_ptr<float>(),
+        dlogits.data_ptr<float>(), dx.data_ptr(), B, K, C, stream.stream());
+    TORCH_CHECK(rc == 0, "head bwd (master) launch failed");
+    return {dlogits, dx};
+}
+
+std::vector<torch::Tensor> head_wgrads(torch::Tensor dlogits,
+                                       torch::Tensor x) {
+    check_f32_cuda(dlogits, "head dlogits");
+    TORCH_CHECK(x.is_cuda() && x.is_contiguous() && x.dim() == 2 &&
+                dlogits.dim() == 2 && dlogits.size(0) == x.size(0),
+                "head_wgrads: shape mismatch");
+    const bool bf16 = compute_dtype_is_bf16(x.scalar_type());
+    const int B = x.size(0), K = x.size(1), C = dlogits.size(1);
+    const int64_t n_slabs = fmda_head_wgrads_slabs(B);
+    auto f32 = dlogits.options();
+    auto dw_part = torch::empty({n_slabs, C, K}, f32);
+    auto db_part = torch::empty({n_slabs, C}, f32);
+    auto dW = torch::empty({C, K}, f32);
+    auto db = torch::empty({C}, f32);
+    auto stream = at::hip::getCurrentHIPStream();
+    int rc = fmda_head_wgrads_launch(
+        bf16 ? 1 : 0, dlogits.data_ptr<float>(), x.data_ptr(),
+        dw_part.data_ptr<float>(), db_part.data_ptr<float>(),
+        dW.data_ptr<float>(), db.data_ptr<float>(), B, K, C,
+        stream.stream());
+    TORCH_CHECK(rc == 0, "head_wgrads launch failed");
+    return {dW, db};
+}
+
 PYBIND11_MODULE(TORCH_EXTENSION_NAME, m) {
     m.def("gru_fwd", &gru_fwd, "fused biGRU recurrence forward (HIP/CDNA4)",
           py::arg("gi"), py::arg("w"), py::arg("bhh"),
@@ -506,7 +720,8 @@
     m.def("gru_bwd", &gru_bwd, "fused biGRU recurrence backward (HIP/CDNA4)",
           py::arg("gi"), py::arg("w"), py::arg("bhh"), py::arg("out"),
           py::arg("dout"), py::arg("dhT"), py::arg("drop_p") = 0.0,
-          py::arg("drop_seed") = 0, py::arg("h0") = py::none());
+          py::arg("drop_seed") = 0, py::arg("h0") = py::none(),
+          py::arg("wt") = py::none());
     m.def("mfma_selftest", &mfma_selftest, "mfma fragment layout self-test");
     m.def("dropout_fused", &dropout_fused,
           "counter-based dropout (mask recomputed in backward)");
@@ -518,10 +733,21 @@
           "fused [dirsum(h_last) | max | avg] concat for inference");
     m.def("head_sigmoid", &head_sigmoid,
           "linear head + sigmoid emitting probabilities");
-    m.def("pool_fwd", &pool_fwd, "fused dirsum+max/avg pooling forward");
+    m.def("pool_fwd", &pool_fwd, "fused dirsum+max/avg pooling forward",
+          py::arg("out"), py::arg("n_dir"), py::arg("act_dtype") = false);
     m.def("pool_bwd", &pool_bwd, "fused pooling backward (d_out assembly)");
     m.def("head_loss_fwd", &head_loss_fwd, "fused head GEMM + BCE loss");
     m.def("head_loss_bwd", &head_loss_bwd, "fused head/loss backward");
+    m.def("pack_gru_layer", &pack_gru_layer,
+          "fp32 masters -> padded compute-dtype layer weights (+ W_hh^T)");
+    m.def("finalize_gru_wgrads", &finalize_gru_wgrads,
+          "split-K partials -> master-shaped fp32 dW_ih / dW_hh");
+    m.def("head_loss_fwd_master", &head_loss_fwd_master,
+          "fused head GEMM + BCE loss reading the fp32 master W / b");
+    m.def("head_loss_bwd_master", &head_loss_bwd_master,
+          "fused head/loss backward reading the fp32 master W");
+    m.def("head_wgrads", &head_wgrads,
+          "head dW / db in fp32, two-stage fixed-order batch reduction");
     m.def("fused_clip_adam", &fused_clip_adam,
           "fused multi-tensor grad-clip + Adam step");
     m.def("save_state_dict_native", &fmda_ckpt::save_state_dict,
diff --git a/fmda_amd/ops/csrc/glue_kernels.hip b/fmda_amd/ops/csrc/glue_kernels.hip
--- /dev/null
+++ b/fmda_amd/ops/csrc/glue_kernels.hip
@@ -0,0 +1,372 @@
+#include <hip/hip_runtime.h>
+#include <hip/hip_bf16.h>
+
+#define FMDA_DEV __device__ __forceinline__
+
+namespace fmda {
+namespace {
+
+#define FMDA_LOG2E 1.4426950408889634f
+
+FMDA_DEV float fast_exp2(float x) { return __builtin_amdgcn_exp2f(x); }
+FMDA_DEV float fast_rcp(float x) { return __builtin_amdgcn_rcpf(x); }
+FMDA_DEV float sigmoidf(float x) {
+    return fast_rcp(1.0f + fast_exp2(-x * FMDA_LOG2E));
+}
+
+template <typename T> FMDA_DEV float to_f32(T v);
+template <> FMDA_DEV float to_f32<float>(float v) { return v; }
+template <> FMDA_DEV float to_f32<__hip_bfloat16>(__hip_bfloat16 v) {
+    return __bfloat162float(v);
+}
+template <typename T> FMDA_DEV T from_f32(float v);
+template <> FMDA_DEV float from_f32<float>(float v) { return v; }
+template <> FMDA_DEV __hip_bfloat16 from_f32<__hip_bfloat16>(float v) {
+    return __float2bfloat16(v);
+}
+template <typename T> FMDA_DEV float round_to(float v) {
+    return to_f32<T>(from_f32<T>(v));
+}
+
+struct GruMasters {
+    const float* w_ih[2];
+    const float* w_hh[2];
+    const float* b_ih[2];
+    const float* b_hh[2];
+};
+
+template <typename T>
+__global__ void pack_gru_layer_kernel(GruMasters m, T* __restrict__ w_ih_cat,
+                                      T* __restrict__ b_ih_cat,
+                                      T* __restrict__ w_hh_cat,
+                                      float* __restrict__ b_hh_cat,
+                                      T* __restrict__ wt, int D, int H,
+                                      int Hp, int F) {
+    const long G3 = 3L * Hp;
+    const long n_ih = (long)D * G3 * F;
+    const long n_hh = (long)D * G3 * Hp;
+    const long n_b = (long)D * G3;
+    const long total = n_ih + 2 * n_hh + 2 * n_b;
+    const long stride = (long)gridDim.x * blockDim.x;
+    for (long i = (long)blockIdx.x * blockDim.x + threadIdx.x; i < total;
+         i += stride) {
+        if (i < n_ih) {
+            const int d = (int)(i / (G3 * F));
+            const long rem = i % (G3 * F);
+            const int row = (int)(rem / F), col = (int)(rem % F);
+            const int g = row / Hp, j = row % Hp;
+            const float v =
+                j < H ? m.w_ih[d][((long)g * H + j) * F + col] : 0.0f;
+            w_ih_cat[i] = from_f32<T>(v);
+        } else if (i < n_ih + n_hh) {
+            const long o = i - n_ih;
+            const int d = (int)(o / (G3 * Hp));
+            const long rem = o % (G3 * Hp);
+            const int row = (int)(rem / Hp), col = (int)(rem % Hp);
+            const int g = row / Hp, j = row % Hp;
+            const float v = (j < H && col < H)
+                ? m.w_hh[d][((long)g * H + j) * H + col] : 0.0f;
+            w_hh_cat[o] = from_f32<T>(v);
+        } else if (i < n_ih + 2 * n_hh) {
+            const long o = i - n_ih - n_hh;
+            const int d = (int)(o / (G3 * Hp));
+            const long rem = o % (G3 * Hp);
+            const int k = (int)(rem / G3), n = (int)(rem % G3);
+            const int g = n / Hp, j = n % Hp;
+            const float v = (j < H && k < H)
+                ? m.w_hh[d][((long)g * H + j) * H + k] : 0.0f;
+            wt[o] = from_f32<T>(v);
+        } else {
+            long o = i - n_ih - 2 * n_hh;
+            const bool hh = o >= n_b;
+            if (hh) o -= n_b;
+            const int d = (int)(o / G3);
+            const int row = (int)(o % G3);
+            const int g = row / Hp, j = row % Hp;
+            const float* src = hh ? m.b_hh[d] : m.b_ih[d];
+            const float v = j < H ? src[g * H + j] : 0.0f;
+            if (hh) b_hh_cat[o] = v;
+            else b_ih_cat[o] = from_f32<T>(v);
+        }
+    }
+}
+
+struct GruWgrads {
+    float* dw_ih[2];
+    float* dw_hh[2];
+};
+
+template <typename PT>
+__global__ void finalize_gru_wgrads_kernel(const PT* __restrict__ part_ih,
+                                           int c_ih,
+                                           const PT* __restrict__ part_hh,
+                                           int c_hh, GruWgrads o, int D,
+                                           int H, int Hp, int F) {
+    const long n_ih = 3L * H * F;
+    const long n_hh = 3L * H * H;
+    const long per_dir = n_ih + n_hh;
+    const long idx = (long)blockIdx.x * blockDim.x + threadIdx.x;
+    if (idx >= (long)D * per_dir) return;
+    const int d = (int)(idx / per_dir);
+    const long r = idx % per_dir;
+    float acc = 0.0f;
+    if (r < n_ih) {
+        const int row = (int)(r / F), col = (int)(r % F);
+        const long prow = (long)d * 3 * Hp + (long)(row / H) * Hp + row % H;
+        const PT* p = part_ih + prow * F + col;
+        const long cs = (long)D * 3 * Hp * F;
+#pragma unroll 8
+        for (int k = 0; k < c_ih; ++k) acc += to_f32<PT>(p[k * cs]);
+        o.dw_ih[d][r] = acc;
+    } else {
+        const long q = r - n_ih;
+        const int row = (int)(q / H), col = (int)(q % H);
+        const long prow = (long)d * 3 * Hp + (long)(row / H) * Hp + row % H;
+        const long pitch = (long)D * Hp;
+        const PT* p = part_hh + prow * pitch + (long)d * Hp + col;
+        const long cs = (long)D * 3 * Hp * pitch;
+#pragma unroll 8
+        for (int k = 0; k < c_hh; ++k) acc += to_f32<PT>(p[k * cs]);
+        o.dw_hh[d][q] = acc;
+    }
+}
+
+template <typename T>
+__global__ void head_fwd_master_kernel(const T* __restrict__ x,
+                                       const float* __restrict__ W,
+                                       const float* __restrict__ bias,
+                                       const float* __restrict__ y,
+                                       const float* __restrict__ wgt,
+                                       const float* __restrict__ pw,
+                                       float* __restrict__ logits,
+                                       float* __restrict__ sig,
+                                       float* __restrict__ loss_sum, int B,
+                                       int K, int C) {
+    const int idx = blockIdx.x * blockDim.x + threadIdx.x;
+    float l = 0.0f;
+    if (idx < B * C) {
+        const int r = idx / C, c = idx % C;
+        const T* xr = x + (long)r * K;
+        const float* wr = W + (long)c * K;
+        float acc = round_to<T>(bias[c]);
+        for (int k = 0; k < K; ++k)
+            acc += to_f32<T>(xr[k]) * round_to<T>(wr[k]);
+        logits[idx] = acc;
+        const float s = sigmoidf(acc);
+        sig[idx] = s;
+        const float yy = y[idx];
+        const float m = acc > 0.0f ? acc : 0.0f;
+        const float lse = m + __builtin_logf(fast_exp2(-m * FMDA_LOG2E) +
+                                             fast_exp2((acc - m) * FMDA_LOG2E));
+        const float log_s = acc - lse;
+        const float log_1ms = -lse;
+        l = -wgt[c] * (pw[c] * yy * log_s + (1.0f - yy) * log_1ms);
+    }
+    __shared__ float red[4];
+    float v = l;
+    v += __shfl_xor(v, 1); v += __shfl_xor(v, 2); v += __shfl_xor(v, 4);
+    v += __shfl_xor(v, 8); v += __shfl_xor(v, 16); v += __shfl_xor(v, 32);
+    if ((threadIdx.x & 63) == 0) red[threadIdx.x >> 6] = v;
+    __syncthreads();
+    if (threadIdx.x == 0) {
+        float t = 0.0f;
+        for (int w = 0; w < (int)(blockDim.x >> 6); ++w) t += red[w];
+        loss_sum[blockIdx.x] = t;
+    }
+}
+
+template <typename T>
+__global__ void head_bwd_master_kernel(const float* __restrict__ sig,
+                                       const float* __restrict__ y,
+                                       const float* __restrict__ wgt,
+                                       const float* __restrict__ pw,
+                                       const float* __restrict__ gscale,
+                                       const float* __restrict__ W,
+                                       float* __restrict__ dlogits,
+                                       T* __restrict__ dx, int B, int K,
+                                       int C) {
+    const int idx = blockIdx.x * blockDim.x + threadIdx.x;
+    if (idx >= B * K) return;
+    const int r = idx / K, k = idx % K;
+    const float g = *gscale / (float)(B * C);
+    float acc = 0.0f;
+    for (int c = 0; c < C; ++c) {
+        const float s = sig[r * C + c];
+        const float yy = y[r * C + c];
+        const float dl = g * wgt[c] * (s * (1.0f - yy + pw[c] * yy) -
+                                       pw[c] * yy);
+        if (k == 0) dlogits[r * C + c] = dl;
+        acc += dl * round_to<T>(W[(long)c * K + k]);
+    }
+    dx[idx] = from_f32<T>(acc);
+}
+
+constexpr int HEAD_SLAB = 64;
+
+struct CompSum {
+    float s = 0.0f, c = 0.0f;
+    FMDA_DEV void add(float v) {
+#pragma clang fp contract(off)
+        const float t = s + v;
+        c += fabsf(s) >= fabsf(v) ? (s - t) + v : (v - t) + s;
+        s = t;
+    }
+    FMDA_DEV float value() const { return s + c; }
+};
+
+template <typename T>
+__global__ void head_wgrads_stage1_kernel(const float* __restrict__ dlogits,
+                                          const T* __restrict__ x,
+                                          float* __restrict__ dw_part,
+                                          float* __restrict__ db_part, int B,
+                                          int K, int C) {
+    const int k = blockIdx.x * blockDim.x + threadIdx.x;
+    if (k >= K) return;
+    const int slab = blockIdx.y, c = blockIdx.z;
+    const int r0 = slab * HEAD_SLAB;
+    const int r1 = min(r0 + HEAD_SLAB, B);
+    CompSum dw, db;
+#pragma unroll 8
+    for (int r = r0; r < r1; ++r) {
+#pragma clang fp contract(off)
+        const float dl32 = dlogits[(long)r * C + c];
+        const float dl = round_to<T>(dl32);
+        const float xv = to_f32<T>(x[(long)r * K + k]);
+        const float p = dl * xv;
+        dw.add(p);
+        dw.c += __builtin_fmaf(dl, xv, -p);
+        db.add(dl32);
+    }
+    dw_part[((long)slab * C + c) * K + k] = dw.value();
+    if (k == 0) db_part[slab * C + c] = db.value();
+}
+
+__global__ void head_wgrads_stage2_kernel(const float* __restrict__ dw_part,
+                                          const float* __restrict__ db_part,
+                                          float* __restrict__ dW,
+                                          float* __restrict__ db, int n_slabs,
+                                          int K, int C) {
+    const int idx = blockIdx.x * blockDim.x + threadIdx.x;
+    const int n_w = C * K;
+    if (idx >= n_w + C) return;
+    CompSum a;
+    if (idx < n_w) {
+#pragma unroll 8
+        for (int s = 0; s < n_slabs; ++s) a.add(dw_part[(long)s * n_w + idx]);
+        dW[idx] = a.value();
+    } else {
+        const int c = idx - n_w;
+        for (int s = 0; s < n_slabs; ++s) a.add(db_part[s * C + c]);
+        db[c] = a.value();
+    }
+}
+
+inline int launch_ok() { return hipGetLastError() == hipSuccess ? 0 : -1; }
+
+}
+}
+
+using namespace fmda;
+
+extern "C" int fmda_pack_gru_layer_launch(
+        int is_bf16, const float* const* masters, void* w_ih_cat,
+        void* b_ih_cat, void* w_hh_cat, float* b_hh_cat, void* wt, int D,
+        int H, int Hp, int F, hipStream_t stream) {
+    GruMasters m = {};
+    for (int d = 0; d < D; ++d) {
+        m.w_ih[d] = masters[4 * d + 0];
+        m.w_hh[d] = masters[4 * d + 1];
+        m.b_ih[d] = masters[4 * d + 2];
+        m.b_hh[d] = masters[4 * d + 3];
+    }
+    const long total = (long)D * 3 * Hp * ((long)F + 2L * Hp + 2);
+    const long blocks = (total + 255) / 256;
+    const dim3 grid((unsigned)(blocks < 2048 ? blocks : 2048));
+    if (is_bf16)
+        pack_gru_layer_kernel<__hip_bfloat16><<<grid, 256, 0, stream>>>(
+            m, (__hip_bfloat16*)w_ih_cat, (__hip_bfloat16*)b_ih_cat,
+            (__hip_bfloat16*)w_hh_cat, b_hh_cat, (__hip_bfloat16*)wt, D, H,
+            Hp, F);
+    else
+        pack_gru_layer_kernel<float><<<grid, 256, 0, stream>>>(
+            m, (float*)w_ih_cat, (float*)b_ih_cat, (float*)w_hh_cat,
+            b_hh_cat, (float*)wt, D, H, Hp, F);
+    return launch_ok();
+}
+
+extern "C" int fmda_finalize_gru_wgrads_launch(
+        int part_bf16, const void* part_ih, int c_ih, const void* part_hh,
+        int c_hh, float* const* grads, int D, int H, int Hp, int F,
+        hipStream_t stream) {
+    GruWgrads o = {};
+    for (int d = 0; d < D; ++d) {
+        o.dw_ih[d] = grads[2 * d + 0];
+        o.dw_hh[d] = grads[2 * d + 1];
+    }
+    const long total = (long)D * 3 * H * ((long)F + H);
+    const dim3 grid((unsigned)((total + 255) / 256));
+    if (part_bf16)
+        finalize_gru_wgrads_kernel<__hip_bfloat16><<<grid, 256, 0, stream>>>(
+            (const __hip_bfloat16*)part_ih, c_ih,
+            (const __hip_bfloat16*)part_hh, c_hh, o, D, H, Hp, F);
+    else
+        finalize_gru_wgrads_kernel<float><<<grid, 256, 0, stream>>>(
+            (const float*)part_ih, c_ih, (const float*)part_hh, c_hh, o, D,
+            H, Hp, F);
+    return launch_ok();
+}
+
+extern "C" int fmda_head_fwd_master_launch(
+        int is_bf16, const void* x, const float* W, const float* bias,
+        const float* y, const float* wgt, const float* pw, float* logits,
+        float* sig, float* loss_sum, int B, int K, int C,
+        hipStream_t stream) {
+    const dim3 grid((B * C + 255) / 256);
+    if (is_bf16)
+        head_fwd_master_kernel<__hip_bfloat16><<<grid, 256, 0, stream>>>(
+            (const __hip_bfloat16*)x, W, bias, y, wgt, pw, logits, sig,
+            loss_sum, B, K, C);
+    else
+        head_fwd_master_kernel<float><<<grid, 256, 0, stream>>>(
+            (const float*)x, W, bias, y, wgt, pw, logits, sig, loss_sum, B,
+            K, C);
+    return launch_ok();
+}
+
+extern "C" int fmda_head_bwd_master_launch(
+        int is_bf16, const float* sig, const float* y, const float* wgt,
+        const float* pw, const float* gscale, const float* W,
+        float* dlogits, void* dx, int B, int K, int C, hipStream_t stream) {
+    const dim3 grid((B * K + 255) / 256);
+    if (is_bf16)
+        head_bwd_master_kernel<__hip_bfloat16><<<grid, 256, 0, stream>>>(
+            sig, y, wgt, pw, gscale, W, dlogits, (__hip_bfloat16*)dx, B, K,
+            C);
+    else
+        head_bwd_master_kernel<float><<<grid, 256, 0, stream>>>(
+            sig, y, wgt, pw, gscale, W, dlogits, (float*)dx, B, K, C);
+    return launch_ok();
+}
+
+extern "C" int fmda_head_wgrads_slabs(int B) {
+    return (B + HEAD_SLAB - 1) / HEAD_SLAB;
+}
+
+extern "C" int fmda_head_wgrads_launch(
+        int is_bf16, const float* dlogits, const void* x, float* dw_part,
+        float* db_part, float* dW, float* db, int B, int K, int C,
+        hipStream_t stream) {
+    const int n_slabs = fmda_head_wgrads_slabs(B);
+    const dim3 grid1((K + 127) / 128, n_slabs, C);
+    if (is_bf16)
+        head_wgrads_stage1_kernel<__hip_bfloat16><<<grid1, 128, 0, stream>>>(
+            dlogits, (const __hip_bfloat16*)x, dw_part, db_part, B, K, C);
+    else
+        head_wgrads_stage1_kernel<float><<<grid1, 128, 0, stream>>>(
+            dlogits, (const float*)x, dw_part, db_part, B, K, C);
+    if (launch_ok() != 0) return -1;
+    const dim3 grid2((C * K + C + 255) / 256);
+    head_wgrads_stage2_kernel<<<grid2, 256, 0, stream>>>(
+        dw_part, db_part, dW, db, n_slabs, K, C);
+    return launch_ok();
+}
diff --git a/fmda_amd/ops/csrc/gru_kernels.hip b/fmda_amd/ops/csrc/gru_kernels.hip
--- a/fmda_amd/ops/csrc/gru_kernels.hip
+++ b/fmda_amd/ops/csrc/gru_kernels.hip
@@ -2251,10 +2251,10 @@
     return hipGetLastError() == hipSuccess ? 0 : -1;
 }
 
-template <typename T>
+template <typename T, typename OT>
 __global__ void pool_fwd_kernel(const T* __restrict__ out,
-                                float* __restrict__ maxv,
-                                float* __restrict__ avgv,
+                                OT* __restrict__ maxv,
+                                OT* __restrict__ avgv,
                                 int* __restrict__ amax, int B, int Tseq,
                                 int H, int n_dir) {
     const int idx = blockIdx.x * blockDim.x + threadIdx.x;
@@ -2281,24 +2281,25 @@
         if (v1 > mx1) { mx1 = v1; im1 = t; }
     }
     const int o = b * H + h2;
-    maxv[o] = mx0; maxv[o + 1] = mx1;
-    avgv[o] = s0 / (float)Tseq; avgv[o + 1] = s1 / (float)Tseq;
+    maxv[o] = from_f32<OT>(mx0); maxv[o + 1] = from_f32<OT>(mx1);
+    avgv[o] = from_f32<OT>(s0 / (float)Tseq);
+    avgv[o + 1] = from_f32<OT>(s1 / (float)Tseq);
     amax[o] = im0; amax[o + 1] = im1;
 }
 
-template <typename T>
-__global__ void pool_bwd_kernel(const float* __restrict__ dmax,
-                                const float* __restrict__ davg,
+template <typename T, typename GT>
+__global__ void pool_bwd_kernel(const GT* __restrict__ dmax,
+                                const GT* __restrict__ davg,
                                 const int* __restrict__ amax,
                                 T* __restrict__ dout, int B, int Tseq, int H,
-                                int n_dir) {
+                                int n_dir, long ld_max, long ld_avg) {
     const int idx = blockIdx.x * blockDim.x + threadIdx.x;
     if (idx >= B * H) return;
     const int b = idx / H;
     const int h = idx % H;
     const int HD = n_dir * H;
-    const float ga = davg[idx] / (float)Tseq;
-    const float gm = dmax[idx];
+    const float ga = to_f32<GT>(davg[b * ld_avg + h]) / (float)Tseq;
+    const float gm = to_f32<GT>(dmax[b * ld_max + h]);
     const int im = amax[idx];
     T* p = dout + (long)b * Tseq * HD + h;
     for (int t = 0; t < Tseq; ++t) {
@@ -2308,9 +2309,10 @@
     }
 }
 
+template <typename OT>
 __global__ void pool_fwd_oct_kernel(const __hip_bfloat16* __restrict__ out,
-                                    float* __restrict__ maxv,
-                                    float* __restrict__ avgv,
+                                    OT* __restrict__ maxv,
+                                    OT* __restrict__ avgv,
                                     int* __restrict__ amax, int B, int Tseq,
                                     int H, int n_dir) {
     const int idx = blockIdx.x * blockDim.x + threadIdx.x;
@@ -2340,17 +2342,19 @@
     const int o = b * H + h8;
 #pragma unroll
     for (int k = 0; k < 8; ++k) {
-        maxv[o + k] = mx[k];
-        avgv[o + k] = s[k] / (float)Tseq;
+        maxv[o + k] = from_f32<OT>(mx[k]);
+        avgv[o + k] = from_f32<OT>(s[k] / (float)Tseq);
         amax[o + k] = im[k];
     }
 }
 
-__global__ void pool_bwd_oct_kernel(const float* __restrict__ dmax,
-                                    const float* __restrict__ davg,
+template <typename GT>
+__global__ void pool_bwd_oct_kernel(const GT* __restrict__ dmax,
+                                    const GT* __restrict__ davg,
                                     const int* __restrict__ amax,
                                     __hip_bfloat16* __restrict__ dout,
-                                    int B, int Tseq, int H, int n_dir) {
+                                    int B, int Tseq, int H, int n_dir,
+                                    long ld_max, long ld_avg) {
     const int idx = blockIdx.x * blockDim.x + threadIdx.x;
     const int H8 = H / 8;
     if (idx >= B * H8) return;
@@ -2361,8 +2365,8 @@
     int im[8];
 #pragma unroll
     for (int k = 0; k < 8; ++k) {
-        ga[k] = davg[o + k] / (float)Tseq;
-        gm[k] = dmax[o + k];
+        ga[k] = to_f32<GT>(davg[b * ld_avg + h8 + k]) / (float)Tseq;
+        gm[k] = to_f32<GT>(dmax[b * ld_max + h8 + k]);
         im[k] = amax[o + k];
     }
     const int HD = n_dir * H;
@@ -2378,10 +2382,10 @@
     }
 }
 
-template <typename T>
+template <typename T, typename OT>
 __global__ void pool_fwd_small_kernel(const T* __restrict__ out,
-                                      float* __restrict__ maxv,
-                                      float* __restrict__ avgv,
+                                      OT* __restrict__ maxv,
+                                      OT* __restrict__ avgv,
                                       int* __restrict__ amax, int B, int Tseq,
                                       int H, int n_dir) {
     const int HP2 = H / 2;
@@ -2420,61 +2424,99 @@
     }
     if (lane == 0) {
         const int o = b * H + h2;
-        maxv[o] = mx0; maxv[o + 1] = mx1;
-        avgv[o] = s0 / (float)Tseq; avgv[o + 1] = s1 / (float)Tseq;
+        maxv[o] = from_f32<OT>(mx0); maxv[o + 1] = from_f32<OT>(mx1);
+        avgv[o] = from_f32<OT>(s0 / (float)Tseq);
+        avgv[o + 1] = from_f32<OT>(s1 / (float)Tseq);
         amax[o] = im0; amax[o + 1] = im1;
     }
 }
 
-extern "C" int fmda_pool_fwd_launch(int is_bf16, const void* out, float* maxv,
-                                    float* avgv, int* amax, int B, int Tseq,
-                                    int H, int n_dir, hipStream_t stream) {
+extern "C" int fmda_pool_fwd_launch(int is_bf16, const void* out, void* maxv,
+                                    void* avgv, int* amax, int B, int Tseq,
+                                    int H, int n_dir, int act_io,
+                                    hipStream_t stream) {
+    using bf16 = __hip_bfloat16;
+    if (act_io && !is_bf16) return -2;
     const int n = B * (H / 2);
     if (n < 4096) {
         const dim3 grid((n + 3) / 4);
-        if (is_bf16)
-            pool_fwd_small_kernel<__hip_bfloat16><<<grid, 256, 0, stream>>>(
-                (const __hip_bfloat16*)out, maxv, avgv, amax, B, Tseq, H,
+        if (act_io)
+            pool_fwd_small_kernel<bf16, bf16><<<grid, 256, 0, stream>>>(
+                (const bf16*)out, (bf16*)maxv, (bf16*)avgv, amax, B, Tseq, H,
+                n_dir);
+        else if (is_bf16)
+            pool_fwd_small_kernel<bf16, float><<<grid, 256, 0, stream>>>(
+                (const bf16*)out, (float*)maxv, (float*)avgv, amax, B, Tseq,
+                H, n_dir);
+        else
+            pool_fwd_small_kernel<float, float><<<grid, 256, 0, stream>>>(
+                (const float*)out, (float*)maxv, (float*)avgv, amax, B, Tseq,
+                H, n_dir);
+        return hipGetLastError() == hipSuccess ? 0 : -1;
+    }
+    if (is_bf16 && H % 8 == 0) {
+        const int n8 = B * (H / 8);
+        const dim3 grid8((n8 + 255) / 256);
+        if (act_io)
+            pool_fwd_oct_kernel<bf16><<<grid8, 256, 0, stream>>>(
+                (const bf16*)out, (bf16*)maxv, (bf16*)avgv, amax, B, Tseq, H,
                 n_dir);
         else
-            pool_fwd_small_kernel<float><<<grid, 256, 0, stream>>>(
-                (const float*)out, maxv, avgv, amax, B, Tseq, H, n_dir);
+            pool_fwd_oct_kernel<float><<<grid8, 256, 0, stream>>>(
+                (const bf16*)out, (float*)maxv, (float*)avgv, amax, B, Tseq,
+                H, n_dir);
         return hipGetLastError() == hipSuccess ? 0 : -1;
     }
-    if (is_bf16 && H % 8 == 0) {
-        const int n8 = B * (H / 8);
-        pool_fwd_oct_kernel<<<dim3((n8 + 255) / 256), 256, 0, stream>>>(
-            (const __hip_bfloat16*)out, maxv, avgv, amax, B, Tseq, H, n_dir);
-        return hipGetLastError() == hipSuccess ? 0 : -1;
-    }
     const dim3 grid((n + 255) / 256);
-    if (is_bf16)
-        pool_fwd_kernel<__hip_bfloat16><<<grid, 256, 0, stream>>>(
-            (const __hip_bfloat16*)out, maxv, avgv, amax, B, Tseq, H, n_dir);
+    if (act_io)
+        pool_fwd_kernel<bf16, bf16><<<grid, 256, 0, stream>>>(
+            (const bf16*)out, (bf16*)maxv, (bf16*)avgv, amax, B, Tseq, H,
+            n_dir);
+    else if (is_bf16)
+        pool_fwd_kernel<bf16, float><<<grid, 256, 0, stream>>>(
+            (const bf16*)out, (float*)maxv, (float*)avgv, amax, B, Tseq, H,
+            n_dir);
     else
-        pool_fwd_kernel<float><<<grid, 256, 0, stream>>>(
-            (const float*)out, maxv, avgv, amax, B, Tseq, H, n_dir);
+        pool_fwd_kernel<float, float><<<grid, 256, 0, stream>>>(
+            (const float*)out, (float*)maxv, (float*)avgv, amax, B, Tseq, H,
+            n_dir);
     return hipGetLastError() == hipSuccess ? 0 : -1;
 }
 
-extern "C" int fmda_pool_bwd_launch(int is_bf16, const float* dmax,
-                                    const float* davg, const int* amax,
+extern "C" int fmda_pool_bwd_launch(int is_bf16, const void* dmax,
+                                    const void* davg, const int* amax,
                                     void* dout, int B, int Tseq, int H,
-                                    int n_dir, hipStream_t stream) {
+                                    int n_dir, int act_io, long ld_max,
+                                    long ld_avg, hipStream_t stream) {
+    using bf16 = __hip_bfloat16;
+    if (act_io && !is_bf16) return -2;
     const int n = B * H;
     if (is_bf16 && H % 8 == 0 && B * (H / 8) >= 4096) {
         const int n8 = B * (H / 8);
-        pool_bwd_oct_kernel<<<dim3((n8 + 255) / 256), 256, 0, stream>>>(
-            dmax, davg, amax, (__hip_bfloat16*)dout, B, Tseq, H, n_dir);
+        const dim3 grid8((n8 + 255) / 256);
+        if (act_io)
+            pool_bwd_oct_kernel<bf16><<<grid8, 256, 0, stream>>>(
+                (const bf16*)dmax, (const bf16*)davg, amax, (bf16*)dout, B,
+                Tseq, H, n_dir, ld_max, ld_avg);
+        else
+            pool_bwd_oct_kernel<float><<<grid8, 256, 0, stream>>>(
+                (const float*)dmax, (const float*)davg, amax, (bf16*)dout, B,
+                Tseq, H, n_dir, ld_max, ld_avg);
         return hipGetLastError() == hipSuccess ? 0 : -1;
     }
     const dim3 grid((n + 255) / 256);
-    if (is_bf16)
-        pool_bwd_kernel<__hip_bfloat16><<<grid, 256, 0, stream>>>(
-            dmax, davg, amax, (__hip_bfloat16*)dout, B, Tseq, H, n_dir);
+    if (act_io)
+        pool_bwd_kernel<bf16, bf16><<<grid, 256, 0, stream>>>(
+            (const bf16*)dmax, (const bf16*)davg, amax, (bf16*)dout, B, Tseq,
+            H, n_dir, ld_max, ld_avg);
+    else if (is_bf16)
+        pool_bwd_kernel<bf16, float><<<grid, 256, 0, stream>>>(
+            (const float*)dmax, (const float*)davg, amax, (bf16*)dout, B,
+            Tseq, H, n_dir, ld_max, ld_avg);
     else
-        pool_bwd_kernel<float><<<grid, 256, 0, stream>>>(
-            dmax, davg, amax, (float*)dout, B, Tseq, H, n_dir);
+        pool_bwd_kernel<float, float><<<grid, 256, 0, stream>>>(
+            (const float*)dmax, (const float*)davg, amax, (float*)dout, B,
+            Tseq, H, n_dir, ld_max, ld_avg);
     return hipGetLastError() == hipSuccess ? 0 : -1;
 }
 
diff --git a/fmda_amd/ops/interface.py b/fmda_amd/ops/interface.py
--- a/fmda_amd/ops/interface.py
+++ b/fmda_amd/ops/interface.py
@@ -4,7 +4,8 @@
 import torch
 
 from . import load_extension
-from .blas import chunked_colsum, chunked_outer, enable_tunableop
+from .blas import (chunked_colsum, chunked_outer, chunked_outer_parts,
+                   enable_tunableop)
 
 _ALLOWED_HP = [32, 64, 128, 256, 512]
 
@@ -14,6 +15,22 @@
         if H <= hp:
             return hp
     raise ValueError(f"hidden size {H} > {_ALLOWED_HP[-1]} not supported")
+
+
+def _glue_mode() -> int:
+    return {"0": 0, "2": 2}.get(os.environ.get("FMDA_NATIVE_GLUE", "1"), 1)
+
+
+def _native_glue() -> bool:
+    return _glue_mode() >= 1
+
+
+def _native_reductions() -> bool:
+    return _glue_mode() == 2
+
+
+def _fp32_cuda(*tensors) -> bool:
+    return all(t.is_cuda and t.dtype == torch.float32 for t in tensors)
 
 
 def _pad_gate_rows(w: torch.Tensor, H: int, Hp: int) -> torch.Tensor:
@@ -35,6 +52,28 @@
     out = w.new_zeros(shape)
     out[..., :H] = w
     return out
+
+
+def _pack_layer_eager(params, H: int, Hp: int, dtype):
+    w_ihs, w_hhs, b_ihs, b_hhs = [], [], [], []
+    for (w_ih, w_hh, b_ih, b_hh) in params:
+        w_ihs.append(_pad_gate_rows(w_ih, H, Hp))
+        w_hhs.append(_pad_cols(_pad_gate_rows(w_hh, H, Hp), H, Hp))
+        b_ihs.append(_pad_gate_rows(b_ih, H, Hp))
+        b_hhs.append(_pad_gate_rows(b_hh, H, Hp))
+    return (torch.cat(w_ihs, dim=0).to(dtype),
+            torch.cat(b_ihs, dim=0).to(dtype),
+            torch.stack(w_hhs, dim=0).to(dtype).contiguous(),
+            torch.stack(b_hhs, dim=0).float().contiguous())
+
+
+def _pack_layer(params, H: int, Hp: int, dtype):
+    flat = [t for four in params for t in four]
+    if (_native_glue() and _fp32_cuda(*flat)
+            and dtype in (torch.bfloat16, torch.float32)):
+        return tuple(load_extension().pack_gru_layer(
+            [t.detach().contiguous() for t in flat], Hp, dtype))
+    return _pack_layer_eager(params, H, Hp, dtype) + (None,)
 
 
 class _GRURecurrence(torch.autograd.Function):
@@ -157,18 +196,24 @@
     def forward(ctx, out, n_dir):
         ext = load_extension()
         out = out.contiguous()
-        maxv, avgv, amax = ext.pool_fwd(out, n_dir)
+        native = _native_glue()
+        maxv, avgv, amax = ext.pool_fwd(out, n_dir, native)
         ctx.save_for_backward(amax)
-        ctx.meta = (out.shape[1], n_dir, out.dtype)
+        ctx.meta = (out.shape[1], n_dir, out.dtype, native)
         return maxv.to(out.dtype), avgv.to(out.dtype)
 
     @staticmethod
     def backward(ctx, dmax, davg):
         ext = load_extension()
         (amax,) = ctx.saved_tensors
-        T, n_dir, dtype = ctx.meta
-        dout = ext.pool_bwd(dmax.float().contiguous(),
-                            davg.float().contiguous(), amax, T, n_dir, dtype)
+        T, n_dir, dtype, native = ctx.meta
+        if native and dmax.dtype == dtype and davg.dtype == dtype:
+            if any(g.stride(1) != 1 or g.stride(0) < g.shape[1]
+                   for g in (dmax, davg)):
+                dmax, davg = dmax.contiguous(), davg.contiguous()
+        else:
+            dmax, davg = dmax.float().contiguous(), davg.float().contiguous()
+        dout = ext.pool_bwd(dmax, davg, amax, T, n_dir, dtype)
         return dout, None
 
 
@@ -204,7 +249,43 @@
         return dx, dW, db, None, None, None
 
 
+class _HeadLossMaster(torch.autograd.Function):
+
+    @staticmethod
+    def forward(ctx, x2d, W, b, y, wgt, pw):
+        ext = load_extension()
+        ctx.native_reductions = _native_reductions()
+        x2d = x2d.contiguous()
+        W = W.contiguous()
+        y, wgt, pw = y.contiguous(), wgt.contiguous(), pw.contiguous()
+        logits, sig, loss_sum = ext.head_loss_fwd_master(
+            x2d, W, b.contiguous(), y, wgt, pw)
+        B, C = logits.shape
+        loss = (loss_sum / float(B * C)).reshape(())
+        ctx.save_for_backward(x2d, W, y, wgt, pw, sig)
+        ctx.mark_non_differentiable(logits)
+        return loss, logits
+
+    @staticmethod
+    def backward(ctx, dloss, _dlogits):
+        ext = load_extension()
+        x2d, W, y, wgt, pw, sig = ctx.saved_tensors
+        dlogits, dx = ext.head_loss_bwd_master(
+            sig, y, wgt, pw, dloss.reshape(1).float().contiguous(), W,
+            x2d.dtype)
+        if ctx.native_reductions:
+            dW, db = ext.head_wgrads(dlogits, x2d)
+        else:
+            dW = chunked_outer(dlogits.to(x2d.dtype), x2d).to(W.dtype)
+            db = dlogits.sum(dim=0).to(x2d.dtype).to(W.dtype)
+        return dx, dW, db, None, None, None
+
+
 def fused_head_loss(x2d, weight, bias, y, wgt, pw):
+    if (_native_glue() and x2d.is_cuda and _fp32_cuda(weight, bias)
+            and x2d.dtype in (torch.bfloat16, torch.float32)):
+        return _HeadLossMaster.apply(x2d, weight, bias, y.float(),
+                                     wgt.float(), pw.float())
     Wc = weight.to(x2d.dtype)
     bc = bias.to(x2d.dtype)
     return _HeadLoss.apply(x2d, Wc, bc, y.float(), wgt.float(), pw.float())
@@ -227,29 +308,22 @@
         H = w_hh0.shape[1]
         dtype = x.dtype
         B, T, F = x.shape
+        params = [(w_ih0, w_hh0, b_ih0, b_hh0)]
+        if D == 2:
+            params.append((w_ih1, w_hh1, b_ih1, b_hh1))
         with torch.no_grad():
-            w_ihs = [_pad_gate_rows(w_ih0, H, Hp)]
-            w_hhs = [_pad_cols(_pad_gate_rows(w_hh0, H, Hp), H, Hp)]
-            b_ihs = [_pad_gate_rows(b_ih0, H, Hp)]
-            b_hhs = [_pad_gate_rows(b_hh0, H, Hp)]
-            if D == 2:
-                w_ihs.append(_pad_gate_rows(w_ih1, H, Hp))
-                w_hhs.append(_pad_cols(_pad_gate_rows(w_hh1, H, Hp), H, Hp))
-                b_ihs.append(_pad_gate_rows(b_ih1, H, Hp))
-                b_hhs.append(_pad_gate_rows(b_hh1, H, Hp))
-            w_ih_cat = torch.cat(w_ihs, dim=0).to(dtype)
-            b_ih_cat = torch.cat(b_ihs, dim=0).to(dtype)
-            w_hh_cat = torch.stack(w_hhs, dim=0).to(dtype)
-            b_hh_cat = torch.stack(b_hhs, dim=0).float()
+            w_ih_cat, b_ih_cat, w_hh_cat, b_hh_cat, wt = _pack_layer(
+                params, H, Hp, dtype)
         x2d = x.reshape(B * T, F)
         gi = torch.addmm(b_ih_cat, x2d, w_ih_cat.t()).view(B, T, -1)
         h0c = h0.detach().contiguous() if h0 is not None else None
         res = ext.gru_fwd(gi, w_hh_cat, b_hh_cat, h0c, out_drop_p,
                           out_drop_seed)
         out, h_last = res[0], res[1]
-        ctx.save_for_backward(x2d, w_ih_cat, w_hh_cat, b_hh_cat, gi, out)
+        ctx.save_for_backward(x2d, w_ih_cat, w_hh_cat, b_hh_cat, gi, out, wt)
         ctx.h0 = h0c
         ctx.meta = (D, H, Hp, out_drop_p, out_drop_seed)
+        ctx.native_reductions = _native_reductions()
         ctx.set_materialize_grads(False)
         if len(res) > 2:
             return out, h_last, res[2]
@@ -258,7 +332,7 @@
     @staticmethod
     def backward(ctx, d_out, d_hlast, d_outdrop=None):
         ext = load_extension()
-        x2d, w_ih_cat, w_hh_cat, b_hh_cat, gi, out = ctx.saved_tensors
+        x2d, w_ih_cat, w_hh_cat, b_hh_cat, gi, out, wt = ctx.saved_tensors
         D, H, Hp, drop_p, drop_seed = ctx.meta
         need_dx = ctx.needs_input_grad[0]
         if drop_p > 0:
@@ -273,37 +347,44 @@
         d_hlast = d_hlast.contiguous().float()
         h0c = ctx.h0
         res = ext.gru_bwd(gi, w_hh_cat, b_hh_cat, out, d_out, d_hlast,
-                          drop_p, drop_seed, h0c)
+                          drop_p, drop_seed, h0c, wt)
         dgi, dgh, dh0_out, dbhh, dbih = res[:5]
         dgh0 = res[5] if len(res) > 5 else None
         M = dgi.shape[0] * dgi.shape[1]
-
-        cross = chunked_outer(dgh.reshape(M, -1), out.reshape(M, -1),
-                              out_fp32=True)
-        if dgh0 is not None:
-            for d in range(D):
-                cross[d * 3 * Hp:(d + 1) * 3 * Hp,
-                      d * Hp:(d + 1) * Hp] += dgh0[d].float().t() @ h0c[d]
-        dwih_cat = chunked_outer(dgi.reshape(M, -1), x2d, out_fp32=True)
         dx = None
         if need_dx:
             dx = torch.matmul(dgi.reshape(M, -1), w_ih_cat)
             dx = dx.view(dgi.shape[0], dgi.shape[1], -1)
-
-        grads = []
-        for d in range(D):
-            dwih = dwih_cat[d * 3 * Hp:(d + 1) * 3 * Hp]
-            dwhh = cross[d * 3 * Hp:(d + 1) * 3 * Hp,
-                         d * Hp:(d + 1) * Hp].contiguous()
-            grads.append((
-                _unpad_gate_rows(dwih, H, Hp),
-                _unpad_gate_rows(dwhh, H, Hp)[:, :H],
-                _unpad_gate_rows(dbih[d], H, Hp),
-                _unpad_gate_rows(dbhh[d], H, Hp)))
+        dh0_grad = dh0_out if h0c is not None else None
+
+        if wt is not None and ctx.native_reductions and dgh0 is None:
+            wg = ext.finalize_gru_wgrads(
+                chunked_outer_parts(dgi.reshape(M, -1), x2d),
+                chunked_outer_parts(dgh.reshape(M, -1), out.reshape(M, -1)),
+                D, H, Hp)
+            wgrads = [(wg[2 * d], wg[2 * d + 1]) for d in range(D)]
+        else:
+            cross = chunked_outer(dgh.reshape(M, -1), out.reshape(M, -1),
+                                  out_fp32=True)
+            if dgh0 is not None:
+                for d in range(D):
+                    cross[d * 3 * Hp:(d + 1) * 3 * Hp,
+                          d * Hp:(d + 1) * Hp] += dgh0[d].float().t() @ h0c[d]
+            dwih_cat = chunked_outer(dgi.reshape(M, -1), x2d, out_fp32=True)
+            wgrads = []
+            for d in range(D):
+                dwih = dwih_cat[d * 3 * Hp:(d + 1) * 3 * Hp]
+                dwhh = cross[d * 3 * Hp:(d + 1) * 3 * Hp,
+                             d * Hp:(d + 1) * Hp].contiguous()
+                wgrads.append((_unpad_gate_rows(dwih, H, Hp),
+                               _unpad_gate_rows(dwhh, H, Hp)[:, :H]))
+
+        grads = [wgrads[d] + (_unpad_gate_rows(dbih[d], H, Hp),
+                              _unpad_gate_rows(dbhh[d], H, Hp))
+                 for d in range(D)]
         if D == 1:
             grads.append((None, None, None, None))
         (a0, b0, c0, e0), (a1, b1, c1, e1) = grads
-        dh0_grad = dh0_out if h0c is not None else None
         return (dx, None, a0, b0, c0, e0, a1, b1, c1, e1, None, None,
                 dh0_grad)
 
@@ -319,16 +400,7 @@
     ent = getattr(gru_module, key, None)
     if ent is not None and ent[0] == versions:
         return ent[1]
-    w_ihs, w_hhs, b_ihs, b_hhs = [], [], [], []
-    for (w_ih, w_hh, b_ih, b_hh) in params:
-        w_ihs.append(_pad_gate_rows(w_ih, H, Hp))
-        w_hhs.append(_pad_cols(_pad_gate_rows(w_hh, H, Hp), H, Hp))
-        b_ihs.append(_pad_gate_rows(b_ih, H, Hp))
-        b_hhs.append(_pad_gate_rows(b_hh, H, Hp))
-    packed = (torch.cat(w_ihs, dim=0).to(dtype),
-              torch.cat(b_ihs, dim=0).to(dtype),
-              torch.stack(w_hhs, dim=0).to(dtype).contiguous(),
-              torch.stack(b_hhs, dim=0).float().contiguous())
+    packed = _pack_layer(params, H, Hp, dtype)[:4]
     setattr(gru_module, key, (versions, packed))
     return packed
 
diff --git a/setup.py b/setup.py
--- a/setup.py
+++ b/setup.py
@@ -17,6 +17,7 @@
             sources=[
                 "fmda_amd/ops/csrc/bindings.cpp",
                 "fmda_amd/ops/csrc/gru_kernels.hip",
+                "fmda_amd/ops/csrc/glue_kernels.hip",
                 "fmda_amd/ops/csrc/optim_kernels.hip",
                 "fmda_amd/ops/csrc/checkpoint.cpp",
             ],
```

Result: faster. 1.082 million seq/s, median of 6 (+2.6%).
